# NingZhang1/pyscf_isdf

Hardware: AMD Instinct MI355X
Metric: isdf_build_plus_get_jk_wall_time (lower is better)
Workload: dtype f64

## Files before the change

### include/mi355_isdf.h

```cpp
#ifndef MI355_ISDF_H
#define MI355_ISDF_H

#include <stdint.h>

#ifdef __cplusplus
extern "C" {
#endif

typedef struct isdf_ctx* isdf_handle;

#define ISDF_OK 0
#define ISDF_ERR_ARG 1
#define ISDF_ERR_HIP 2
#define ISDF_ERR_LIB 3
#define ISDF_ERR_NUM 4

int isdf_abi_version(void);

int isdf_create(int device_id, isdf_handle* out);
int isdf_destroy(isdf_handle h);
int isdf_set_stream(isdf_handle h, void* hip_stream);
const char* isdf_last_error(isdf_handle h);
int64_t isdf_workspace_bytes(isdf_handle h);
int isdf_release_workspace(isdf_handle h);
// ... 58 lines not shown
int isdf_select_ip_gram(isdf_handle h, double* d_A, int m, int64_t ldA, int nip, double tol, double tie_rtol,
                        int panel, int64_t* d_piv, int32_t* rank);

int isdf_select_ip_cplx(isdf_handle h, const double* d_ao, int nao, int nh, int64_t ld,
                        int nblk, const int64_t* blk_off, const int32_t* nip,
                        double tol, double tie_rtol,
                        double* d_L, int64_t ldL, int64_t* d_piv, int32_t* rank);

int isdf_fit_from_chol(isdf_handle h, double* d_L, int k, int64_t m, int64_t ldL,
                       const int64_t* d_piv);

int isdf_fit_prepare(isdf_handle h, const double* d_ao, int nao, int64_t ld,
                     const int64_t* d_ip, int P, double reg_rel, double* d_aoP, double* d_chol,
                     double* reg_used);
int isdf_fit_apply(isdf_handle h, const double* d_chol, const double* d_aoP, int P, int nao,
                   const double* d_ao, int64_t ng, int64_t ld, int forward_only,
                   double* d_theta, int64_t ldt);
int isdf_fit_prepare_cplx(isdf_handle h, const double* d_ao, int nao, int nh, int64_t ld,
                          const int64_t* d_ip, int P, double reg_rel, double* d_aoP, double* d_chol,
                          double* reg_used);
int isdf_fit_apply_cplx(isdf_handle h, const double* d_chol, const double* d_aoP, int P, int nao, int nh,
                        const double* d_ao, int64_t ng, int64_t ld, int forward_only,
                        double* d_theta, int64_t ldt);
int isdf_fit_global(isdf_handle h, const double* d_ao, int nao, int64_t ngrids, int64_t ld,
                    const int64_t* d_ip, int P, double reg_rel, double* d_theta, int64_t ldt,
                    double* d_aoP, double* reg_used);

int isdf_gather_aoP(isdf_handle h, const double* d_ao, int nao, int64_t ld, const int64_t* d_ip, int P,
                    double* d_aoP);
int isdf_gram_sq(isdf_handle h, const double* d_aoP, int P, int nao, int nh, double* d_A);
int isdf_pair_gram_rows(isdf_handle h, const double* d_aoP, int P, int nao, int nh, const double* d_ao,
                        int64_t ng, int64_t ld, double* d_B, int64_t ldb);
int isdf_block_chol(isdf_handle h, const double* d_A, int P, int nblk, const int32_t* blk_off,
                    double shift_rel, double* d_D, double* shift_used);
int isdf_block_solve(isdf_handle h, const double* d_D, int P, int nblk, const int32_t* blk_off, int side,
                     int trans, double* d_X, int64_t n, int64_t ldx);
int isdf_block_invert(isdf_handle h, const double* d_D, int P, int nblk, const int32_t* blk_off, double* d_Dinv);
int isdf_block_apply(isdf_handle h, const double* d_Dinv, int64_t ldd, int nblk, const int32_t* blk_off,
                     double* d_X, int64_t n, int64_t ldx);
int isdf_pair_rows_block_apply(isdf_handle h, const double* d_aoP, int P, int nao, const double* d_ao, int64_t ng,
                               int64_t ld, const double* d_Dinv, int64_t ldd, int nblk, const int32_t* blk_off,
                               double* d_B, int64_t ldb);
int isdf_pair_rows_squared(isdf_handle h, const double* d_aoP, int rows, int nao, const double* d_ao, int64_t ng,
                           int64_t ld, int* squared);
int isdf_pair_rows_frontier(isdf_handle h, const double* d_aoP, int nnew, int nao, const double* d_ao, int64_t ng,
                            int64_t ld, int squared, const double* d_Dinv, int64_t ldd, int nblk, const int32_t* blk_off,
                            double* d_B, int64_t ldb, int have);

int isdf_gram_prod(isdf_handle h, const double* d_aoP, int P, int nao, const double* d_psiP, int nocc, double* d_A);
int isdf_pair_prod_rows(isdf_handle h, const double* d_aoP, int P, int nao, const double* d_psiP, int nocc,
                        const double* d_ao, int64_t ld, const double* d_psi, int64_t ldpsi, int64_t ng,
                        double* d_B, int64_t ldb);
int isdf_factor_solve_half(isdf_handle h, const double* d_fac, int P, int backward, double* d_X, int64_t n, int64_t ldx);
int isdf_gram_prod_cplx(isdf_handle h, const double* d_aoP, int P, int nao, int nh, const double* d_psiP, int npsi, int npsi_h,
                        double* d_A);
int isdf_pair_prod_rows_cplx(isdf_handle h, const double* d_aoP, int P, int nao, int nh, const double* d_psiP, int npsi,
                             int npsi_h, const double* d_ao, int64_t ld, const double* d_psi, int64_t ldpsi, int64_t ng,
                             double* d_B, int64_t ldb);

int isdf_shift_diag(isdf_handle h, double* d_A, int P, double shift_rel);
int isdf_chol_inplace(isdf_handle h, double* d_A, int P, double shift_rel, double* d_scratch, double* reg_used);

int isdf_factor_solve(isdf_handle h, const double* d_fac, int P, double* d_X, int64_t n, int64_t ldx);

int isdf_bj_probe_vectors(isdf_handle h, double* d_T, int n, const double* d_fac, const double* d_D, int P,
                          int nblk, const int32_t* blk_off);
int isdf_rows_combine(isdf_handle h, const double* d_E, int n, int64_t ldE, int rows, const double* d_Y,
                      int64_t ng, int64_t ldy, double* d_F, int64_t ldf, int accumulate);

int isdf_bj_probe_rows(isdf_handle h, double* d_T, int n, const double* d_fac, const double* d_D, int P, int nblk,
                       const int32_t* blk_off, const double* d_Yp, int64_t ng, int64_t ldy, double* d_F, int64_t ldf);

int isdf_gather_T(isdf_handle h, const double* d_L, int k, int64_t ldL, const int64_t* d_piv,
                  double* d_T);
int isdf_W_from_factor(isdf_handle h, const double* d_F, int P, int kind, double* d_M, int64_t ldm);

int isdf_coulomb_W(isdf_handle h, const double* d_theta, int P, int64_t ldt,
                   const int32_t mesh[3], const double a[9],
                   int row0, int nrows, int batch, int upper_only, double* d_W, int64_t ldw);
int isdf_coulG_half(isdf_handle h, const int32_t mesh[3], const double a[9], double* d_out);
int isdf_spectral_supported(isdf_handle h, const int32_t mesh[3], int batch, int* ok);
int isdf_spectral_rows(isdf_handle h, const double* d_in, int nrows, int64_t ld, const int32_t mesh[3], const int32_t* d_idx,
                       const double* d_scale, int npts, int batch, double* d_out, int64_t ldx);
int isdf_coulomb_rows(isdf_handle h, const double* d_in, int nrows, int64_t ld,
                      const int32_t mesh[3], const double a[9], int batch, double* d_out, int64_t ldo);
int isdf_symmetrize_upper(isdf_handle h, double* d_W, int P, int64_t ldw);
int isdf_symmetrize_mean(isdf_handle h, double* d_W, int P, int64_t ldw, int antisymmetric);

int isdf_get_j(isdf_handle h, const double* d_ao, int nao, int64_t ngrids, int64_t ld,
               const int32_t mesh[3], const double a[9],
               const double* d_dm, int nset, double* d_vj);
int isdf_rho(isdf_handle h, const double* d_ao, int nao, int64_t ng, int64_t ld,
             const double* d_dm, int nset, double* d_rho, int64_t ldrho);
int isdf_coulomb_potential(isdf_handle h, double* d_rho_inout, int nset, int64_t ldrho,
                           const int32_t mesh[3], const double a[9]);
int isdf_vj_from_vR(isdf_handle h, const double* d_ao, int nao, int64_t ng, int64_t ld,
                    const double* d_vR, int nset, int64_t ldv, double* d_vj);

int isdf_get_k_exact(isdf_handle h, const double* d_ao, int nao, int64_t ngrids, int64_t ld,
                     const double* d_C, int nocc, const int32_t mesh[3], const double a[9],
                     int i0, int ni, int max_rows, double* d_vk);

int isdf_get_k(isdf_handle h, const double* d_aoP, int P, int nao,
               const double* d_W, int64_t ldw, int row0, int nrows,
               const double* d_dm, int nset, double* d_vk);

int isdf_coulG_q(isdf_handle h, const int32_t mesh[3], const double a[9], const double q[3], int wrap_around,
                 double omega, double* d_out);

int isdf_coulomb_Wq(isdf_handle h, const double* d_theta, int P, int64_t ldt, const int32_t mesh[3],
                    const double* d_coulG, double weight, int row0, int nrows, int batch,
                    int upper_only, double* d_Wre, double* d_Wim, int64_t ldw);
int isdf_symmetrize_hermitian(isdf_handle h, double* d_Wre, double* d_Wim, int P, int64_t ldw);
int isdf_finish_Wq(isdf_handle h, const double* d_Wre, const double* d_Wim, int P, int64_t ldw,
                   const double* d_phase, double* d_Wc);
int isdf_get_k_pair(isdf_handle h, const double* d_A1, const double* d_A2, const double* d_D2,
                    const double* d_Wq, int P, int nao, double scale, double* d_vk);

int isdf_get_k_exact_kpt(isdf_handle h, const double* d_u1r, const double* d_u1i, int nao, int64_t ld1,
                         const double* d_m2r, const double* d_m2i, int nocc, int64_t ld2, const int32_t mesh[3],
                         const double* d_coulG, double weight, int i0, int ni, int max_rows, double* d_vk_re,
                         double* d_vk_im);

int isdf_coulomb_rows_q(isdf_handle h, const double* d_rows, int nrows, int64_t ld, const int32_t mesh[3],
                        const double* d_coulG, double* d_re, double* d_im);
int isdf_nyquist_spectra(isdf_handle h, const double* d_rows, int nrows, int64_t ld, const int32_t mesh[3], int axis,
                         double* d_re, double* d_im);
int isdf_zhadamard_planes(isdf_handle h, double* d_Ar, double* d_Ai, int64_t lda, const double* d_Br, const double* d_Bi,
                          int64_t ldb, int rows, int64_t cols);
int isdf_rho_k(isdf_handle h, const double* d_ur, const double* d_ui, int nao, int64_t ng, int64_t ld,
               const double* d_DTr, const double* d_DTi, double scale, double* d_rho);
int isdf_vj_k(isdf_handle h, const double* d_ur, const double* d_ui, int nao, int64_t ng, int64_t ld,
              const double* d_vR, double* d_vj_re, double* d_vj_im);

int isdf_pp_local_potential(isdf_handle h, int natm, const double* coords, const double* pp_par,
                            const int32_t mesh[3], const double a[9], double* d_vlocR);
int isdf_pp_projector_overlaps(isdf_handle h, const int32_t* atm, int natm, const int32_t* bas, int nbas,
                               const double* env, int nenv, const double* coords, const double kpt[3],
                               const int32_t* proj_tab, const double* proj_rl, int nproj,
                               const int32_t mesh[3], const double a[9], double* d_out);

int isdf_pp_local_force(isdf_handle h, const double* d_rho, int nset, int64_t ldrho, int natm, const double* coords,
                        const double* pp_par, const int32_t mesh[3], const double a[9], double* d_out);
int isdf_pp_projector_overlaps_ip(isdf_handle h, const int32_t* atm, int natm, const int32_t* bas, int nbas,
                                  const double* env, int nenv, const double* coords, const double kpt[3],
                                  const int32_t* proj_tab, const double* proj_rl, int nproj,
                                  const int32_t mesh[3], const double a[9], double* d_out);
int isdf_rowdot3(isdf_handle h, int M, int64_t K, double alpha, const double* d_A, int64_t lda, int64_t astride, const double* d_s,
                 const double* d_B, int64_t ldb, int accumulate, double* d_out, int64_t ldo);
int isdf_gga_aow(isdf_handle h, int M, int64_t K, const double* d_ao, int64_t ld, int64_t plane, const double* d_w, int64_t ldw,
                 double* d_Z, int64_t ldz, double* d_G, int64_t ldg, int64_t gstride);

int isdf_gemm_nn(isdf_handle h, int M, int64_t N, int K, double alpha, const double* d_A, int64_t lda, const double* d_B,
                 int64_t ldb, double beta, double* d_C, int64_t ldc);
int isdf_hadamard_rows(isdf_handle h, double* d_X, int64_t ldx, const double* d_Y, int64_t ldy, int rows, int64_t cols);

int isdf_uniform_grid(isdf_handle h, const int32_t mesh[3], const double a[9], double* d_coords_soa);
int isdf_rho_pair(isdf_handle h, const double* d_aoA, int nA, const double* d_aoB, int nB, int64_t ng, int64_t ld,
                  const double* d_dm, int nset, double* d_rho, int64_t ldrho);
int isdf_mg_embed_density(isdf_handle h, const double* d_field, int nset, const int32_t mesh_sub[3], double scale,
                          double* d_spec, const int32_t mesh[3], int accumulate);
int isdf_mg_restrict_potential(isdf_handle h, const double* d_spec, int nset, const int32_t mesh[3],
                               const int32_t mesh_sub[3], double scale, double* d_field);
int isdf_mg_coulomb_kernel(isdf_handle h, double* d_spec, int nset, const int32_t mesh[3], const double a[9]);
int isdf_lda_exchange(isdf_handle h, const double* d_rho, int64_t n, double* d_exc, double* d_vxc);
int isdf_lda_vwn_add(isdf_handle h, const double* d_rho, int64_t n, double* d_exc, double* d_vxc);
// ... 36 lines not shown
```

### pyscf_isdf_amd/backend.py

```python
import ctypes
import os
import numpy as np
import torch
from . import lib as _lib

_vp = ctypes.c_void_p


def _np_ptr(a):
    return a.ctypes.data_as(_vp)


class HipBackend:
    name = 'hip-gfx950'

    def __init__(self, device=0):
        if not torch.cuda.is_available():
            raise _lib.IsdfError('no GPU visible to torch; the ISDF path has no CPU fallback')
        self.device = torch.device('cuda', device)
        torch.cuda.set_device(self.device)
        self.handle = _lib.Handle(device)
        if os.environ.get('ISDF_TRSM') == 'subst':
            self.set_option('trsm_substitution', 1)
        if os.environ.get('ISDF_OWN_FFT') in ('0', '1', '2'):
# ... 309 lines not shown

    def shift_diag(self, A, shift_rel):
        self._stream()
        self.handle.call('isdf_shift_diag', self._p(A), A.shape[0], float(shift_rel))

    def chol_inplace(self, A, shift_rel, scratch=None):
        self._stream()
        reg = ctypes.c_double(0.0)
        assert scratch is None or scratch.numel() >= A.numel()
        self.handle.call('isdf_chol_inplace', self._p(A), A.shape[0], float(shift_rel),
                         self._p(scratch) if scratch is not None else None, ctypes.byref(reg))
        return reg.value

    def factor_solve(self, fac, X):
        self._stream()
        self.handle.call('isdf_factor_solve', self._p(fac), fac.shape[0], self._p(X), X.shape[1], X.stride(0))

    def bj_probe_rows(self, T, fac, D, blk_off, Yp, ng, F):
        self._stream()
        blk_off = np.ascontiguousarray(blk_off, dtype=np.int32)
        self.handle.call('isdf_bj_probe_rows', self._p(T), T.shape[0], self._p(fac), self._p(D), D.shape[0],
                         len(blk_off) - 1, _np_ptr(blk_off), self._p(Yp), int(ng), Yp.stride(0), self._p(F), F.stride(0))

    def bj_probe_vectors(self, T, fac, D, blk_off):
        self._stream()
        blk_off = np.ascontiguousarray(blk_off, dtype=np.int32)
        assert T.is_contiguous()
        self.handle.call('isdf_bj_probe_vectors', self._p(T), T.shape[0], self._p(fac), self._p(D), D.shape[0],
                         len(blk_off) - 1, _np_ptr(blk_off))

    def rows_combine(self, E, Y, F, accumulate=False):
        self._stream()
        assert E.stride(1) == 1 and Y.stride(1) == 1 and F.stride(1) == 1 and E.shape[1] == Y.shape[0]
        self.handle.call('isdf_rows_combine', self._p(E), E.shape[0], E.stride(0), E.shape[1], self._p(Y), Y.shape[1],
                         Y.stride(0), self._p(F), F.stride(0), int(bool(accumulate)))

    def gather_T(self, L, k, piv, T):
        self._stream()
        assert T.is_contiguous() and T.shape == (k, k)
        self.handle.call('isdf_gather_T', self._p(L), int(k), L.stride(0), self._p(piv), self._p(T))

    def W_from_factor(self, F, kind, M):
        self._stream()
        assert F.is_contiguous()
        self.handle.call('isdf_W_from_factor', self._p(F), M.shape[0], int(kind), self._p(M), M.stride(0))

    def fit_global(self, ao, ngrids, ip, reg_rel, theta, aoP):
        self._stream()
        assert ip.dtype == torch.int64 and aoP.is_contiguous()
        reg = ctypes.c_double(0.0)
        self.handle.call('isdf_fit_global', self._p(ao), ao.shape[0], int(ngrids), ao.stride(0), self._p(ip),
                         ip.numel(), float(reg_rel), self._p(theta), theta.stride(0), self._p(aoP), ctypes.byref(reg))
        return reg.value

    def coulomb_W(self, theta, mesh, a, row0, nrows, batch, W, upper_only=False):
        self._stream()
        mesh = np.ascontiguousarray(mesh, dtype=np.int32)
        a = np.ascontiguousarray(a, dtype=np.float64)
        self.handle.call('isdf_coulomb_W', self._p(theta), theta.shape[0], theta.stride(0), _np_ptr(mesh), _np_ptr(a),
                         int(row0), int(nrows), int(batch), int(bool(upper_only)), self._p(W), W.stride(0))

    def coulomb_rows(self, rows, mesh, a, batch, out=None):
        self._stream()
        out = rows if out is None else out
        mesh = np.ascontiguousarray(mesh, dtype=np.int32)
        a = np.ascontiguousarray(a, dtype=np.float64)
        self.handle.call('isdf_coulomb_rows', self._p(rows), rows.shape[0], rows.stride(0), _np_ptr(mesh), _np_ptr(a),
                         int(batch), self._p(out), out.stride(0))

    def spectral_supported(self, mesh, batch=512):
        ok = ctypes.c_int(0)
        mesh = np.ascontiguousarray(mesh, dtype=np.int32)
        self.handle.call('isdf_spectral_supported', _np_ptr(mesh), int(batch), ctypes.byref(ok))
        return bool(ok.value)

    def coulG_half(self, mesh, a):
        self._stream()
        mesh = np.ascontiguousarray(mesh, dtype=np.int32)
        a = np.ascontiguousarray(a, dtype=np.float64)
        out = self.empty((int(mesh[0]) * int(mesh[1]) * (int(mesh[2]) // 2 + 1),))
        self.handle.call('isdf_coulG_half', _np_ptr(mesh), _np_ptr(a), self._p(out))
        return self.to_host(out).reshape(int(mesh[0]), int(mesh[1]), int(mesh[2]) // 2 + 1)

    def spectral_rows(self, rows, mesh, idx, scale, out, batch=512):
        self._stream()
        mesh = np.ascontiguousarray(mesh, dtype=np.int32)
        assert rows.is_contiguous() and out.stride(1) == 1 and idx.dtype == torch.int32 and out.stride(0) % 2 == 0
        self.handle.call('isdf_spectral_rows', self._p(rows), rows.shape[0], rows.stride(0), _np_ptr(mesh), self._p(idx),
                         self._p(scale), int(idx.numel()), int(batch), self._p(out), out.stride(0))

    def symmetrize_upper(self, W):
        self._stream()
        self.handle.call('isdf_symmetrize_upper', self._p(W), W.shape[0], W.stride(0))

    def symmetrize_mean(self, W, antisymmetric=False):
        self._stream()
        self.handle.call('isdf_symmetrize_mean', self._p(W), W.shape[0], W.stride(0), int(bool(antisymmetric)))

    def get_j(self, ao, ngrids, mesh, a, dm, vj):
        self._stream()
        mesh = np.ascontiguousarray(mesh, dtype=np.int32)
        a = np.ascontiguousarray(a, dtype=np.float64)
        assert dm.is_contiguous() and vj.is_contiguous()
        self.handle.call('isdf_get_j', self._p(ao), ao.shape[0], int(ngrids), ao.stride(0), _np_ptr(mesh), _np_ptr(a),
                         self._p(dm), dm.shape[0], self._p(vj))

    def rho(self, ao, ng, dm, rho):
        self._stream()
        self.handle.call('isdf_rho', self._p(ao), ao.shape[0], int(ng), ao.stride(0), self._p(dm), dm.shape[0],
                         self._p(rho), rho.stride(0))

    def coulomb_potential(self, rho, mesh, a):
        self._stream()
        mesh = np.ascontiguousarray(mesh, dtype=np.int32)
        a = np.ascontiguousarray(a, dtype=np.float64)
        self.handle.call('isdf_coulomb_potential', self._p(rho), rho.shape[0], rho.stride(0), _np_ptr(mesh), _np_ptr(a))

    def vj_from_vR(self, ao, ng, vR, vj):
        self._stream()
        self.handle.call('isdf_vj_from_vR', self._p(ao), ao.shape[0], int(ng), ao.stride(0), self._p(vR), vR.shape[0],
                         vR.stride(0), self._p(vj))

    def get_k(self, aoP, W, row0, nrows, dm, vk):
        self._stream()
        assert aoP.is_contiguous() and dm.is_contiguous() and vk.is_contiguous()
        self.handle.call('isdf_get_k', self._p(aoP), aoP.shape[0], aoP.shape[1], self._p(W), W.stride(0), int(row0),
                         int(nrows), self._p(dm), dm.shape[0], self._p(vk))

    def get_k_exact(self, ao, ngrids, C, mesh, a, i0, ni, max_rows, vk):
        self._stream()
        mesh = np.ascontiguousarray(mesh, dtype=np.int32)
        a = np.ascontiguousarray(a, dtype=np.float64)
        assert C.is_contiguous() and vk.is_contiguous()
        self.handle.call('isdf_get_k_exact', self._p(ao), ao.shape[0], int(ngrids), ao.stride(0), self._p(C), C.shape[1],
                         _np_ptr(mesh), _np_ptr(a), int(i0), int(ni), int(max_rows), self._p(vk))

    def gemm_nn(self, A, B, C, alpha=1.0, beta=0.0):
        self._stream()
        self.handle.call('isdf_gemm_nn', A.shape[0], B.shape[1], A.shape[1], float(alpha), self._p(A), A.stride(0), self._p(B),
                         B.stride(0), float(beta), self._p(C), C.stride(0))

    def hadamard_rows(self, X, Y):
        self._stream()
        self.handle.call('isdf_hadamard_rows', self._p(X), X.stride(0), self._p(Y), Y.stride(0), X.shape[0], X.shape[1])

    def gemm_nt(self, A, B, C, alpha=1.0, beta=0.0, kscale=None):
        self._stream()
        M, K = A.shape
        N = B.shape[0]
        assert B.shape[1] == K and tuple(C.shape) == (M, N) and A.stride(1) == 1 and B.stride(1) == 1 and C.stride(1) == 1
        ks = self._p(kscale) if kscale is not None else _vp(0)
        self.handle.call('isdf_gemm_nt', M, N, K, float(alpha), self._p(A), A.stride(0), self._p(B), B.stride(0), ks,
                         float(beta), self._p(C), C.stride(0))

    def gemm_nt_had3(self, A, H, B3, C3, alpha=1.0, beta=0.0):
        self._stream()
        M, K = A.shape
        N = B3.shape[1]
        assert tuple(B3.shape) == (3, N, K) and tuple(C3.shape) == (3, M, N) and A.stride(1) == 1 and B3.stride(2) == 1 and C3.stride(2) == 1
        assert H is None or (tuple(H.shape) == (M, K) and H.stride(1) == 1)
        self.handle.call('isdf_gemm_nt_had3', M, N, K, float(alpha), self._p(A), A.stride(0), self._p(H) if H is not None else _vp(0),
                         H.stride(0) if H is not None else 0, self._p(B3), B3.stride(1), B3.stride(0), float(beta), self._p(C3),
                         C3.stride(1), C3.stride(0))

    def gemm_nn_had(self, A, H, B, C, alpha=1.0, beta=0.0):
        self._stream()
        M, K = A.shape
        N = B.shape[1]
        assert tuple(B.shape) == (K, N) and tuple(H.shape) == (K, N) and tuple(C.shape) == (M, N)
        assert A.stride(1) == 1 and H.stride(1) == 1 and B.stride(1) == 1 and C.stride(1) == 1
        self.handle.call('isdf_gemm_nn_had', M, N, K, float(alpha), self._p(A), A.stride(0), self._p(H), H.stride(0), self._p(B),
                         B.stride(0), float(beta), self._p(C), C.stride(0))
# ... 283 lines not shown
```

### pyscf_isdf_amd/csrc/common.h

```cpp
#pragma once
#include <hip/hip_runtime.h>
#include <rocblas/rocblas.h>
#include <rocsolver/rocsolver.h>
#include <hipfft/hipfft.h>
#include <cstdint>
#include <cstdio>
#include <cstring>
#include <string>
#include <vector>
#include <map>
#include "../../include/mi355_isdf.h"

struct FftPlan {
  hipfftHandle fwd = 0, bwd = 0;
  size_t work_bytes = 0;
};

struct ProfRec {
  hipEvent_t e0 = nullptr, e1 = nullptr;
};
struct ProfEntry {
  std::vector<ProfRec> recs;
  double work = 0.0;
  double ms = 0.0;
  int64_t launches = 0;
};

struct WsKernel {
  double alpha = 0.0;
  double ak[9] = {0};
  int mesh[3] = {0, 0, 0};
  double maxq[3] = {0, 0, 0};
  const double* vq = nullptr;
};

struct isdf_ctx {
  int profiling = 0;
  std::map<std::string, ProfEntry> prof;
  int device = 0;
  hipStream_t stream = nullptr;
  rocblas_handle blas = nullptr;
  std::string err;
  std::map<std::vector<int>, FftPlan> plans;
  std::map<std::string, std::pair<void*, size_t>> ws;
  int num_cu = 256;
  int trsm_substitution = 0;
  int own_fft = 2;
  int gemm_nn_own = 0;
  int attr_gemm_b = 0, attr_gemm_nn = 0, attr_gemm_nn_had = 0, attr_gram_tri = 0, attr_herm = 0;
  int cand_gram = 1;
  int conv_pipe = 1;
  int conv_sub_rows = 0;
  int gram_pivot_tpb = 256;
  int gram_compact = 1;
  int gram_compact_permille = 875;
  int block_apply_waves = 16;
  int block_apply_reg = 1;
  double coul_omega = 0.0;
  double coul_rc = 0.0;
  int coul_sphere = 0;
  WsKernel wsk;
};

int isdf_fail(isdf_handle h, int code, const char* fmt, ...);
void* isdf_ws(isdf_handle h, const char* name, size_t bytes);
int isdf_get_plan(isdf_handle h, const int32_t mesh[3], int batch, FftPlan** out);
int get_coulG_half(isdf_handle h, const int32_t mesh[3], const double a[9], double extra_scale, double** out);
bool conv_rows_own_supported(const int32_t mesh[3], int nb);
bool conv_rows_q_own_supported(isdf_handle h, const int32_t mesh[3], int nb);
bool spectral_rows_own_supported(isdf_handle h, const int32_t mesh[3], int nb);
int spectral_rows_own(isdf_handle h, const double* d_in, int nb, const int32_t mesh[3], const int32_t* d_idx, const double* d_scale,
                      int npts, double* d_out, int64_t ldx, HIP_vector_type<double, 2u>* zbuf);
int conv_rows_q_own(isdf_handle h, const double* d_in, double* d_re, double* d_im, int nb, const int32_t mesh[3], const double* tab,
                    double2* zhalf, double2* zfull);
int conv_rows_own(isdf_handle h, const double* d_in, double* d_out, int nb, const int32_t mesh[3], const double* cg,
                  double2* zbuf);

#define HIP_TRY(h, expr)                                                                    \
  do {                                                                                      \
    hipError_t e_ = (expr);                                                                 \
    if (e_ != hipSuccess)                                                                   \
      return isdf_fail(h, ISDF_ERR_HIP, "%s:%d %s -> %s", __FILE__, __LINE__, #expr,        \
                       hipGetErrorString(e_));                                              \
  } while (0)
#define BLAS_TRY(h, expr)                                                                   \
  do {                                                                                      \
    rocblas_status s_ = (expr);                                                             \
    if (s_ != rocblas_status_success)                                                       \
      return isdf_fail(h, ISDF_ERR_LIB, "%s:%d %s -> rocblas status %d", __FILE__, __LINE__, \
                       #expr, (int)s_);                                                     \
  } while (0)
#define FFT_TRY(h, expr)                                                                    \
  do {                                                                                      \
    hipfftResult r_ = (expr);                                                               \
    if (r_ != HIPFFT_SUCCESS)                                                               \
      return isdf_fail(h, ISDF_ERR_LIB, "%s:%d %s -> hipfft result %d", __FILE__, __LINE__,  \
                       #expr, (int)r_);                                                     \
  } while (0)
#define KERNEL_CHECK(h) HIP_TRY(h, hipGetLastError())
#define ARG_CHECK(h, cond)                                                                  \
  do {                                                                                      \
    if (!(cond)) return isdf_fail(h, ISDF_ERR_ARG, "%s:%d argument check failed: %s",       \
                                  __FILE__, __LINE__, #cond);                               \
  } while (0)

static inline int64_t cdiv(int64_t a, int64_t b) { return (a + b - 1) / b; }

struct ProfScope {
  isdf_handle h;
  ProfRec rec;
  ProfEntry* ent = nullptr;
  ProfScope(isdf_handle h_, const char* name, double work, int64_t launches = 1) : h(h_) {
    if (!h || !h->profiling) return;
    ent = &h->prof[name];
    ent->work += work;
    ent->launches += launches;
    if (hipEventCreate(&rec.e0) != hipSuccess || hipEventCreate(&rec.e1) != hipSuccess) { ent = nullptr; return; }
    (void)hipEventRecord(rec.e0, h->stream);
  }
  ~ProfScope() {
    if (!ent) return;
    (void)hipEventRecord(rec.e1, h->stream);
    ent->recs.push_back(rec);
  }
};

int gemm_nt_f64(isdf_handle h, int M, int N, int64_t K, double alpha, const double* A, int64_t lda,
                const double* B, int64_t ldb, double beta, double* C, int64_t ldc);
int gemm_nt_f64_scaled(isdf_handle h, int M, int N, int64_t K, double alpha, const double* A, int64_t lda,
                       const double* B, int64_t ldb, const double* kscale, double beta, double* C,
                       int64_t ldc);
int trsm_lower_left(isdf_handle h, bool trans, int m, int64_t n, const double* L, int64_t ldl, double* X, int64_t ldx);
int trsm_lower_right(isdf_handle h, bool trans, int m, int64_t n, const double* L, int64_t ldl, double* X, int64_t ldx);
int block_forward_solve(isdf_handle h, const double* D, int64_t ldd, int nblk, const int32_t* blk_off_host, double* X,
                        int64_t ldx, int64_t n);
int block_apply_inverse(isdf_handle h, const double* Dinv, int64_t ldd, int nblk, const int32_t* blk_off_host, double* X,
                        int64_t ldx, int64_t n, bool square_input = false);
int transpose_rm(isdf_handle h, const double* src, int64_t lds, int64_t rows, int64_t cols, double* dst, int64_t ldd);
int tri_left(isdf_handle h, bool trans, int m, int64_t n, const double* L, int64_t ldl, double* X, int64_t ldx);
int tri_right(isdf_handle h, bool trans, int m, int64_t n, const double* L, int64_t ldl, double* X, int64_t ldx);
bool gemm_nn_f64_supported(isdf_handle h, int64_t M, int64_t N, int64_t K, const double* A, int64_t lda, const double* B,
                           int64_t ldb);
int gemm_nn_f64(isdf_handle h, int64_t M, int64_t N, int64_t K, const double* A, int64_t lda, const double* B, int64_t ldb,
                double* C, int64_t ldc, bool square);
int gemm_rm(isdf_handle h, char opA, char opB, int64_t M, int64_t N, int64_t K, double alpha,
            const double* A, int64_t lda, const double* B, int64_t ldb, double beta, double* C,
            int64_t ldc);

__host__ __device__ inline int64_t gram_tri_row(int64_t r) {
  const int64_t tm = r >> 8;
  return 32768 * tm * (tm + 1) + (r & 255) * ((tm + 1) << 8);
}
static inline int64_t gram_tri_size(int64_t m) { return m > 0 ? gram_tri_row(m - 1) + (((m - 1) >> 8) + 1) * 256 : 0; }
struct GramTriUnit { int blk, tm, tn, pad; };
int gram_tri_blocks(isdf_handle h, const double* X, int64_t ldx, int K, const GramTriUnit* d_units, int64_t nunits,
                    const int64_t* d_blk_off, int64_t row0, const int64_t* d_tri_off, double* S, double flop);
```

### pyscf_isdf_amd/csrc/coulomb.hip

```cpp
#include "common.h"

namespace {

struct Recip { double b[9]; };
__device__ inline double g2_of(int ix, int iy, int iz, int n0, int n1, int n2, const Recip& r) {
  const double fx = (ix < (n0 + 1) / 2) ? ix : ix - n0;
  const double fy = (iy < (n1 + 1) / 2) ? iy : iy - n1;
  const double fz = (iz < (n2 + 1) / 2) ? iz : iz - n2;
  const double gx = fx * r.b[0] + fy * r.b[3] + fz * r.b[6];
  const double gy = fx * r.b[1] + fy * r.b[4] + fz * r.b[7];
  const double gz = fx * r.b[2] + fy * r.b[5] + fz * r.b[8];
  return gx * gx + gy * gy + gz * gz;
}

__device__ inline double range_factor(double g2, double omega) {
  if (omega == 0.0) return 1.0;
  const double e = exp(-0.25 * g2 / (omega * omega));
  return omega > 0.0 ? e : 1.0 - e;
}
__device__ inline double kernel_value(double g2, double omega, double rc) {
  const double fourpi = 4.0 * 3.14159265358979323846;
  if (rc > 0.0) return g2 == 0.0 ? 0.5 * fourpi * rc * rc : fourpi / g2 * (1.0 - cos(sqrt(g2) * rc));
  return g2 == 0.0 ? 0.0 : fourpi / g2 * range_factor(g2, omega);
}
// ... 270 lines not shown
    if (rc) return rc;
  }
  return ISDF_OK;
}

extern "C" int isdf_coulomb_potential(isdf_handle h, double* d_rho, int nset, int64_t ldrho,
                                      const int32_t mesh[3], const double a[9]) {
  if (!h) return ISDF_ERR_ARG;
  ARG_CHECK(h, d_rho && mesh && a && nset > 0);
  const int64_t G = (int64_t)mesh[0] * mesh[1] * mesh[2];
  const int64_t gc = (int64_t)mesh[0] * mesh[1] * (mesh[2] / 2 + 1);
  ARG_CHECK(h, ldrho == G);
  const double det = a[0] * (a[4] * a[8] - a[5] * a[7]) - a[1] * (a[3] * a[8] - a[5] * a[6]) +
                     a[2] * (a[3] * a[7] - a[4] * a[6]);
  double* cg = nullptr;
  int rc = get_coulG_half(h, mesh, a, fabs(det) / (double)G, &cg);
  if (rc) return rc;
  double2* Z = (double2*)isdf_ws(h, "coul_Z", sizeof(double2) * (size_t)nset * gc);
  if (!Z) return ISDF_ERR_HIP;
  return convolve_rows(h, d_rho, d_rho, nset, mesh, cg, Z);
}

extern "C" int isdf_coulomb_rows(isdf_handle h, const double* d_in, int nrows, int64_t ld,
                                 const int32_t mesh[3], const double a[9], int batch, double* d_out,
                                 int64_t ldo) {
  if (!h) return ISDF_ERR_ARG;
  ARG_CHECK(h, d_in && d_out && mesh && a && nrows >= 0 && batch > 0);
  const int64_t G = (int64_t)mesh[0] * mesh[1] * mesh[2];
  const int64_t gc = (int64_t)mesh[0] * mesh[1] * (mesh[2] / 2 + 1);
  ARG_CHECK(h, ld == G && ldo == G);
  if (nrows == 0) return ISDF_OK;
  if (batch > nrows) batch = nrows;
  double* cg = nullptr;
  int rc = get_coulG_half(h, mesh, a, 1.0, &cg);
  if (rc) return rc;
  double2* Z = (double2*)isdf_ws(h, "coul_Z", sizeof(double2) * (size_t)batch * gc);
  if (!Z) return ISDF_ERR_HIP;
  for (int r = 0; r < nrows; r += batch) {
    const int nb = std::min(batch, nrows - r);
    rc = convolve_rows(h, d_in + (int64_t)r * ld, d_out + (int64_t)r * ldo, nb, mesh, cg, Z);
    if (rc) return rc;
  }
  return ISDF_OK;
}

extern "C" int isdf_coulG_half(isdf_handle h, const int32_t mesh[3], const double a[9], double* d_out) {
  if (!h) return ISDF_ERR_ARG;
  ARG_CHECK(h, mesh && a && d_out);
  double* cg = nullptr;
  int rc = get_coulG_half(h, mesh, a, 1.0, &cg);
  if (rc) return rc;
  const int64_t gc = (int64_t)mesh[0] * mesh[1] * (mesh[2] / 2 + 1);
  HIP_TRY(h, hipMemcpyAsync(d_out, cg, sizeof(double) * gc, hipMemcpyDeviceToDevice, h->stream));
  return ISDF_OK;
}

extern "C" int isdf_spectral_supported(isdf_handle h, const int32_t mesh[3], int batch, int* ok) {
  if (!h) return ISDF_ERR_ARG;
  ARG_CHECK(h, mesh && ok && batch > 0);
  *ok = spectral_rows_own_supported(h, mesh, batch) ? 1 : 0;
  return ISDF_OK;
}

extern "C" int isdf_spectral_rows(isdf_handle h, const double* d_in, int nrows, int64_t ld, const int32_t mesh[3],
                                  const int32_t* d_idx, const double* d_scale, int npts, int batch, double* d_out, int64_t ldx) {
  if (!h) return ISDF_ERR_ARG;
  ARG_CHECK(h, d_in && d_out && mesh && d_idx && d_scale && nrows >= 0 && batch > 0 && npts > 0);
  const int64_t G = (int64_t)mesh[0] * mesh[1] * mesh[2];
  const int64_t gc = (int64_t)mesh[0] * mesh[1] * (mesh[2] / 2 + 1);
  ARG_CHECK(h, ld == G && npts <= gc);
  if (nrows == 0) return ISDF_OK;
  if (batch > nrows) batch = nrows;
  if (!spectral_rows_own_supported(h, mesh, batch))
    return isdf_fail(h, ISDF_ERR_ARG, "isdf_spectral_rows: mesh %d x %d x %d is not covered by the plane FFT", mesh[0], mesh[1], mesh[2]);
  double2* Z = (double2*)isdf_ws(h, "coul_Z", sizeof(double2) * (size_t)batch * gc);
  if (!Z) return ISDF_ERR_HIP;
  for (int r = 0; r < nrows; r += batch) {
    const int nb = std::min(batch, nrows - r);
    int rc = spectral_rows_own(h, d_in + (int64_t)r * ld, nb, mesh, d_idx, d_scale, npts, d_out + (int64_t)r * ldx, ldx, Z);
    if (rc) return rc;
  }
  return ISDF_OK;
}
```

### pyscf_isdf_amd/csrc/fft_conv.hip

```cpp
#include "common.h"
#include <type_traits>

namespace {

constexpr int TPB = 256;
constexpr int MAXSTAGE = 12;

struct Axis {
  int n;
  int nstage;
  int radix[MAXSTAGE];
  const double2* tw;
};

__device__ inline double2 cadd(double2 a, double2 b) { return make_double2(a.x + b.x, a.y + b.y); }
__device__ inline double2 csub(double2 a, double2 b) { return make_double2(a.x - b.x, a.y - b.y); }
__device__ inline double2 cmul(double2 a, double2 b) { return make_double2(a.x * b.x - a.y * b.y, a.x * b.y + a.y * b.x); }
template <int SIGN>
__device__ inline double2 mul_si(double2 a) { return SIGN > 0 ? make_double2(-a.y, a.x) : make_double2(a.y, -a.x); }
template <int SIGN>
__device__ inline double2 twid(const double2* __restrict__ tw, int idx) {
  double2 w = tw[idx];
  if (SIGN > 0) w.y = -w.y;
  return w;
// ... 432 lines not shown
    if ((l & 1) == 0) r = make_double2(0.5 * (zk.x + zn.x), 0.5 * (zk.y - zn.y));
    else r = make_double2(0.5 * (zk.y + zn.y), -0.5 * (zk.x - zn.x));
    dstc[c] = r;
  }
}

template <int ZCT>
__global__ __launch_bounds__(TPB) void z_c2r_fast_kernel(const double2* __restrict__ in, double* __restrict__ out,
                                                         int64_t nlines, Axis ax) {
  extern __shared__ double2 lds[];
  const int n = ax.n, nh = n / 2 + 1;
  constexpr int Ls = ZCT + 1;
  double2* x = lds;
  double2* tw = lds + n * Ls;
  for (int k = threadIdx.x; k < n; k += TPB) tw[k] = ax.tw[k];
  const int64_t line0 = (int64_t)blockIdx.x * 2 * ZCT;
  const int nl = (int)min((int64_t)2 * ZCT, nlines - line0);
  const int M = (nl + 1) / 2;
  const double2* src = in + line0 * nh;
  const float inv_nh = 1.0f / (float)nh;
  for (int c = threadIdx.x; c < M * nh; c += TPB) {
    const int m = (int)(((float)c + 0.5f) * inv_nh), k = c - m * nh;
    double2 a = src[(int64_t)(2 * m) * nh + k];
    double2 b = (2 * m + 1 < nl) ? src[(int64_t)(2 * m + 1) * nh + k] : make_double2(0.0, 0.0);
    const bool selfconj = (k == 0) || (2 * k == n);
    if (selfconj) { a.y = 0.0; b.y = 0.0; }
    x[k * Ls + m] = make_double2(a.x - b.y, a.y + b.x);
    if (!selfconj) x[(n - k) * Ls + m] = make_double2(a.x + b.y, -a.y + b.x);
  }
  __syncthreads();
  fft_fast<1, ZCT>(x, ax, Ls, tw);
  double* dst = out + line0 * n;
  const float inv_n = 1.0f / (float)n;
  for (int c = threadIdx.x; c < nl * n; c += TPB) {
    const int l = (int)(((float)c + 0.5f) * inv_n), e = c - l * n;
    dst[c] = ((const double*)(x + e * Ls + (l >> 1)))[l & 1];
  }
}

template <int MODE, int ZCT>
__global__ __launch_bounds__(TPB) void strided_fft_fast_kernel(double2* __restrict__ data, int64_t os, int64_t es, int Mtot,
                                                               Axis ax, int ntile, const double* __restrict__ table) {
  extern __shared__ double2 lds[];
  const int n = ax.n;
  double2* x = lds;
  double2* tw = lds + n * ZCT;
  for (int k = threadIdx.x; k < n; k += TPB) tw[k] = ax.tw[k];
  const int nouter = gridDim.x / ntile;
  const int64_t outer = (MODE == 2) ? blockIdx.x % nouter : blockIdx.x / ntile;
  const int m0 = (int)((MODE == 2) ? blockIdx.x / nouter : blockIdx.x % ntile) * ZCT;
  const int M = min(ZCT, Mtot - m0);
  double2* base = data + outer * os + m0;
  for (int c = threadIdx.x; c < n * ZCT; c += TPB) {
    const int e = c / ZCT, m = c & (ZCT - 1);
    if (m < M) x[c] = base[(int64_t)e * es + m];
  }
  __syncthreads();
  if (MODE == 1) {
    fft_fast<1, ZCT>(x, ax, ZCT, tw);
  } else {
    fft_fast<-1, ZCT>(x, ax, ZCT, tw);
    if (MODE == 2) {
      const double* tb = table + m0;
      for (int c = threadIdx.x; c < n * ZCT; c += TPB) {
        const int e = c / ZCT, m = c & (ZCT - 1);
        if (m < M) {
          const double g = tb[(int64_t)e * es + m];
          double2 v = x[c];
          v.x *= g;
          v.y *= g;
          x[c] = v;
        }
      }
      __syncthreads();
      fft_fast<1, ZCT>(x, ax, ZCT, tw);
    }
  }
  for (int c = threadIdx.x; c < n * ZCT; c += TPB) {
    const int e = c / ZCT, m = c & (ZCT - 1);
    if (m < M) base[(int64_t)e * es + m] = x[c];
  }
}

constexpr int TPBP = 1024;
constexpr int PLANE_ENTRIES = 10240;
constexpr int PIPE_NT = 768;

template <int SIGN, int NT, int N, int RA, int RB, int MMAX>
__device__ __forceinline__ void fft_plane_fixed(double2* buf, int Ls, int M, const double2* tw) {
  static_assert(RA * RB == N, "two stages");
  stage<SIGN, RA, NT, ((N / RA) * MMAX + NT - 1) / NT, true, AnyLines>(buf, N, N, 1, Ls, M, tw, opaque_tid());
  stage<SIGN, RB, NT, ((N / RB) * MMAX + NT - 1) / NT, true, AnyLines>(buf, N, N / RA, RA, Ls, M, tw, opaque_tid());
}

struct PlaneAny {
  static constexpr int NT = TPBP, PER = PLANE_ENTRIES / TPBP;
  static constexpr int KS_HALF = PER, KS_PAIR = PER / 2 + 1, KS_FULL = PER;
  int n1, n2, n2h, npair;
  __device__ PlaneAny(const Axis& az, const Axis& ay) : n1(ay.n), n2(az.n), n2h(az.n / 2 + 1), npair((ay.n + 1) / 2) {}
  __device__ static int tid() { return threadIdx.x; }
  template <int SIGN, bool FULL>
  __device__ __forceinline__ static void transform(double2* buf, const Axis& ax, int Ls, int M, const double2* tw) {
    fft<SIGN, NT, PER, false, AnyLines>(buf, ax, Ls, M, tw);
  }
};
template <int N, int RA, int RB>
struct PlaneSquare {
  static constexpr int NT = PIPE_NT, n1 = N, n2 = N, n2h = N / 2 + 1, npair = (N + 1) / 2;
  static constexpr int KS_HALF = (n1 * n2h + NT - 1) / NT, KS_PAIR = (npair * n2h + NT - 1) / NT, KS_FULL = (N * N + NT - 1) / NT;
  constexpr PlaneSquare() = default;
  __device__ static int tid() { return opaque_tid(); }
  template <int SIGN, bool FULL>
  __device__ __forceinline__ static void transform(double2* buf, const Axis&, int Ls, int M, const double2* tw) {
    fft_plane_fixed<SIGN, NT, N, RA, RB, FULL ? N : N / 2 + 1>(buf, Ls, M, tw);
  }
};

__device__ inline double zero_of(const double*) { return 0.0; }
__device__ inline double2 zero_of(const double2*) { return make_double2(0.0, 0.0); }
template <int NT, int NPRE, class T>
__device__ __forceinline__ void prefetch(T (&pre)[NPRE], const T* __restrict__ src, int count, int tid) {
#pragma unroll
  for (int u = 0; u < NPRE; ++u) {
    const int c = tid + u * NT;
    pre[u] = c < count ? src[c] : zero_of(src);
  }
}

template <class D>
__device__ __forceinline__ void plane_fwd_body(const D d, double2* lds, int Lz, int bufsz, const Axis& az, const Axis& ay,
                                               double2* __restrict__ dst, double2 (&r)[D::KS_HALF]) {
  double2* x = lds;
  const double2* twz = lds + bufsz;
  const double2* twy = twz + d.n2;
  d.template transform<-1, false>(x, az, Lz, d.npair, twz);
  int tid = D::tid();
  const float inv_nh = 1.0f / (float)d.n2h;
#pragma unroll
  for (int u = 0; u < D::KS_HALF; ++u) {
    const int c = tid + u * D::NT;
    if (c < d.n1 * d.n2h) {
      const int l = fdiv(c, inv_nh), k = c - l * d.n2h;
      const int m = l >> 1;
      r[u] = separate_pair(x[k * Lz + m], x[(k == 0 ? 0 : d.n2 - k) * Lz + m], l & 1);
    }
  }
  __syncthreads();
#pragma unroll
  for (int u = 0; u < D::KS_HALF; ++u) {
    const int c = tid + u * D::NT;
    if (c < d.n1 * d.n2h) x[c] = r[u];
  }
  __syncthreads();
  d.template transform<-1, false>(x, ay, d.n2h, d.n2h, twy);
  tid = D::tid();
  for (int c = tid; c < d.n1 * d.n2h; c += D::NT) dst[c] = x[c];
}

template <class D>
__device__ __forceinline__ void plane_inv_body(const D d, double2* lds, int Lz, int bufsz, const Axis& az, const Axis& ay,
                                               double* __restrict__ dst, double2 (&za)[D::KS_PAIR], double2 (&zb)[D::KS_PAIR]) {
  double2* x = lds;
  const double2* twz = lds + bufsz;
  const double2* twy = twz + d.n2;
  d.template transform<1, false>(x, ay, d.n2h, d.n2h, twy);
  int tid = D::tid();
// ... 451 lines not shown

int conv_rows_own(isdf_handle h, const double* d_in, double* d_out, int nb, const int32_t mesh[3], const double* cg,
                  double2* zbuf) {
  const int n0 = mesh[0], n1 = mesh[1], n2 = mesh[2], n2h = n2 / 2 + 1;
  Axis ax[3];
  if (int rc = make_axes(h, mesh, ax, "conv_rows_own")) return rc;
  const int64_t gc = (int64_t)n0 * n1 * n2h;
  const int64_t nlines = (int64_t)nb * n0 * n1;
  ARG_CHECK(h, nlines * 4 < 2147483647LL && (int64_t)nb * cdiv((int64_t)n1 * n2h, 1) < 2147483647LL);
  const int LP = lines_per_tile(n2, 1);
  const int ZY = lines_per_tile(n1, 0), ZX = lines_per_tile(n0, 0);
  if (LP < 1 || ZY < 1 || ZX < 1) return isdf_fail(h, ISDF_ERR_ARG, "conv_rows_own: mesh too large for the LDS tiles");
  const int64_t G = (int64_t)n0 * n1 * n2;
  const int FZ = fast_lines(n2), FY = fast_lines(n1), FX = fast_lines(n0);
  const bool smooth = smooth235(ax[0]) && smooth235(ax[1]) && smooth235(ax[2]);
  const PlaneGeo geo = (h->own_fft == 2 && smooth && FX >= 1) ? plane_geometry(n1, n2, false) : PlaneGeo{0, 0, 0};
  ProfScope ps(h, geo.bytes ? "coulomb_conv_own_3pass[byte]" : "coulomb_conv_own_5pass[byte]", 32.0 * (double)G * nb,
               geo.bytes ? 3 : 5);
  if (geo.bytes) {
    const int sub = h->conv_sub_rows > 0 ? std::min(nb, h->conv_sub_rows) : nb;
    for (int r0 = 0; r0 < nb; r0 += sub) {
      const int nr = std::min(sub, nb - r0);
      double2* zb = zbuf + (int64_t)r0 * gc;
      const int nplanes = (int)((int64_t)nr * n0);
      if (int rc = launch_plane_fwd(h, d_in + (int64_t)r0 * G, zb, ax, geo, nplanes, PIPE_ANY)) return rc;
      launch_strided<2>(h, true, FX, zb, nr, gc, (int64_t)n1 * n2h, n1 * n2h, ax[0], cg);
      if (int rc = launch_plane_inv(h, zb, d_out + (int64_t)r0 * G, ax, geo, nplanes, PIPE_ANY)) return rc;
    }
    KERNEL_CHECK(h);
    return ISDF_OK;
  }
  const bool fast = smooth && FZ >= 1 && FY >= 1 && FX >= 1;
  const int Lz = fast ? FZ : LP, Ly = fast ? FY : ZY, Lx = fast ? FX : ZX;
  launch_z<true>(h, fast, Lz, d_in, zbuf, nlines, ax[2]);
  launch_strided<0>(h, fast, Ly, zbuf, (int64_t)nb * n0, (int64_t)n1 * n2h, (int64_t)n2h, n2h, ax[1], nullptr);
  launch_strided<2>(h, fast, Lx, zbuf, nb, gc, (int64_t)n1 * n2h, n1 * n2h, ax[0], cg);
  launch_strided<1>(h, fast, Ly, zbuf, (int64_t)nb * n0, (int64_t)n1 * n2h, (int64_t)n2h, n2h, ax[1], nullptr);
  launch_z<false>(h, fast, Lz, zbuf, d_out, nlines, ax[2]);
  KERNEL_CHECK(h);
  return ISDF_OK;
}

__global__ void spectral_pack_kernel(const double2* __restrict__ z, int64_t gc, const int32_t* __restrict__ idx,
                                     const double* __restrict__ scale, int npts, double2* __restrict__ out, int64_t ldx2) {
  const int64_t j = (int64_t)blockIdx.x * blockDim.x + threadIdx.x;
  if (j >= ldx2) return;
  const int row = blockIdx.y;
  double2 v = make_double2(0.0, 0.0);
  if (j < npts) {
    const double2 t = z[(int64_t)row * gc + idx[j]];
    const double s = scale[j];
    v = make_double2(t.x * s, t.y * s);
  }
  out[(int64_t)row * ldx2 + j] = v;
}

bool spectral_rows_own_supported(isdf_handle h, const int32_t mesh[3], int nb) {
  if (h->own_fft != 2 || !conv_rows_own_supported(mesh, nb)) return false;
  Axis ax[3];
  for (int d = 0; d < 3; ++d)
    if (!factorise(mesh[d], &ax[d]) || !smooth235(ax[d])) return false;
  return fast_lines(mesh[0]) >= 1 && plane_geometry(mesh[1], mesh[2], false).bytes != 0;
}

int spectral_rows_own(isdf_handle h, const double* d_in, int nb, const int32_t mesh[3], const int32_t* d_idx,
                      const double* d_scale, int npts, double* d_out, int64_t ldx, double2* zbuf) {
  const int n0 = mesh[0], n1 = mesh[1], n2 = mesh[2], n2h = n2 / 2 + 1;
  Axis ax[3];
  if (int rc = make_axes(h, mesh, ax, "spectral_rows_own")) return rc;
  const int64_t gc = (int64_t)n0 * n1 * n2h;
  const PlaneGeo geo = plane_geometry(n1, n2, false);
  const int FX = fast_lines(n0);
  ARG_CHECK(h, geo.bytes && FX >= 1 && (int64_t)nb * n0 < 2147483647LL && nb <= 65535 && (ldx & 1) == 0 && ldx >= 2 * (int64_t)npts);
  ProfScope ps(h, "spectral_rows_own[byte]", (8.0 * (double)n0 * n1 * n2 + 8.0 * (double)ldx) * nb, 3);
  if (int rc = launch_plane_fwd(h, d_in, zbuf, ax, geo, (int)((int64_t)nb * n0), PIPE_ANY)) return rc;
  launch_strided<0>(h, true, FX, zbuf, nb, gc, (int64_t)n1 * n2h, n1 * n2h, ax[0], nullptr);
  const int64_t ldx2 = ldx / 2;
  spectral_pack_kernel<<<dim3((unsigned)cdiv(ldx2, 256), (unsigned)nb), dim3(256), 0, h->stream>>>(zbuf, gc, d_idx, d_scale, npts,
                                                                                                  (double2*)d_out, ldx2);
  KERNEL_CHECK(h);
  return ISDF_OK;
}

bool conv_rows_q_own_supported(isdf_handle h, const int32_t mesh[3], int nb) {
  if (!h->own_fft) return false;
  if (nb < 1 || nb > 65535 || (int64_t)nb * mesh[0] >= 2147483647LL) return false;
  Axis ax[3];
  for (int d = 0; d < 3; ++d)
    if (mesh[d] < 2 || mesh[d] > 1024 || !factorise(mesh[d], &ax[d]) || !smooth235(ax[d])) return false;
  return fast_lines(mesh[0]) >= 1 && plane_geometry(mesh[1], mesh[2], false).bytes && plane_geometry(mesh[1], mesh[2], true).bytes;
}

int conv_rows_q_own(isdf_handle h, const double* d_in, double* d_re, double* d_im, int nb, const int32_t mesh[3],
                    const double* tab, double2* zhalf, double2* zfull) {
  const int n0 = mesh[0], n1 = mesh[1], n2 = mesh[2], n2h = n2 / 2 + 1;
  Axis ax[3];
  if (int rc = make_axes(h, mesh, ax, "conv_rows_q_own")) return rc;
  const int64_t G = (int64_t)n0 * n1 * n2, gc = (int64_t)n0 * n1 * n2h;
  const PlaneGeo geo_r = plane_geometry(n1, n2, false), geo_c = plane_geometry(n1, n2, true);
  const int FX = fast_lines(n0);
  ARG_CHECK(h, geo_r.bytes && geo_c.bytes && FX >= 1 && (int64_t)nb * n0 < 2147483647LL && nb <= 65535);
  ProfScope ps(h, "coulomb_conv_q_own[byte]", 64.0 * (double)G * nb, 5);
  const int nplanes = (int)((int64_t)nb * n0);
  if (int rc = launch_plane_fwd(h, d_in, zhalf, ax, geo_r, nplanes, PIPE_Q_MAX)) return rc;
  launch_strided<0>(h, true, FX, zhalf, nb, gc, (int64_t)n1 * n2h, n1 * n2h, ax[0], nullptr);
  expand_mul_kernel<<<dim3((unsigned)cdiv(G, 256), (unsigned)nb), dim3(256), 0, h->stream>>>(zhalf, zfull, tab, n0, n1, n2,
                                                                                            1.0 / (double)G);
  launch_strided<1>(h, true, FX, zfull, nb, G, (int64_t)n1 * n2, n1 * n2, ax[0], nullptr);
  if (int rc = launch_plane_c2c_inv(h, zfull, d_re, d_im, ax, geo_c, nplanes)) return rc;
  KERNEL_CHECK(h);
  return ISDF_OK;
}
```

### pyscf_isdf_amd/csrc/fit.hip

```cpp
#include "common.h"
#include <cstdlib>

namespace {

__global__ void gather_T_kernel(const double* __restrict__ L, int64_t ldL,
                                const int64_t* __restrict__ piv, int k, double* __restrict__ T) {
  const int s = blockIdx.x * blockDim.x + threadIdx.x;
  const int t = blockIdx.y;
  if (s >= k) return;
  T[(int64_t)t * k + s] = (s >= t) ? L[(int64_t)t * ldL + piv[s]] : 0.0;
}

__global__ void square_kernel(double* __restrict__ x, int64_t rows, int64_t cols, int64_t ld) {
  const int64_t c = (int64_t)blockIdx.x * blockDim.x + threadIdx.x;
  const int64_t r = blockIdx.y;
  if (c >= cols) return;
  const double v = x[r * ld + c];
  x[r * ld + c] = v * v;
}

__global__ void square_add_kernel(double* __restrict__ x, int64_t ld, const double* __restrict__ y, int64_t ldy,
                                  int64_t cols) {
  const int64_t c = (int64_t)blockIdx.x * blockDim.x + threadIdx.x;
  const int64_t r = blockIdx.y;
// ... 279 lines not shown
    }
    __syncthreads();
    if (live) {
      const double* y = Y + (int64_t)p0 * ldy + g;
#pragma unroll 8
      for (int pp = 0; pp < np; ++pp) {
        const double v = y[(int64_t)pp * ldy];
#pragma unroll
        for (int j = 0; j < 8; ++j) acc[j] = fma(sE[j][pp], v, acc[j]);
      }
    }
  }
  if (live)
    for (int j = 0; j < n; ++j) F[(int64_t)j * ldf + g] = accumulate ? F[(int64_t)j * ldf + g] + acc[j] : acc[j];
}

__global__ void add_diag_const_kernel(double* __restrict__ A, int n, int64_t ld, double v) {
  const int i = blockIdx.x * blockDim.x + threadIdx.x;
  if (i < n) A[(int64_t)i * ld + i] += v;
}
}

extern "C" int isdf_block_chol(isdf_handle h, const double* d_A, int P, int nblk, const int32_t* blk_off,
                               double shift_rel, double* d_D, double* shift_used) {
  if (!h) return ISDF_ERR_ARG;
  ARG_CHECK(h, d_A && d_D && blk_off && P > 0 && nblk > 0 && blk_off[0] == 0 && blk_off[nblk] == P && shift_rel >= 0);
  int* info = (int*)isdf_ws(h, "fit_info", 256);
  if (!info) return ISDF_ERR_HIP;
  double* maxdiag = (double*)(info + 16);
  HIP_TRY(h, hipMemsetAsync(d_D, 0, sizeof(double) * (size_t)P * P, h->stream));
  hipLaunchKernelGGL(max_diag_kernel, dim3(1), dim3(256), 0, h->stream, d_A, P, maxdiag);
  double md = 0.0;
  HIP_TRY(h, hipMemcpyAsync(&md, maxdiag, sizeof(double), hipMemcpyDeviceToHost, h->stream));
  HIP_TRY(h, hipStreamSynchronize(h->stream));
  double worst = 0.0;
  for (int b = 0; b < nblk; ++b) {
    const int off = blk_off[b], nb = blk_off[b + 1] - off;
    if (nb <= 0) continue;
    ARG_CHECK(h, nb <= 65535);
    double reg = shift_rel;
    int h_info = 1;
    for (int attempt = 0; attempt < 6 && h_info != 0; ++attempt) {
      hipLaunchKernelGGL(copy_block_kernel, dim3((unsigned)cdiv(nb, 128), (unsigned)nb), dim3(128), 0, h->stream, d_A, P,
                         off, nb, d_D);
      if (reg > 0)
        hipLaunchKernelGGL(add_diag_const_kernel, dim3((unsigned)cdiv(nb, 256)), dim3(256), 0, h->stream,
                           d_D + (int64_t)off * P + off, nb, (int64_t)P, reg * md);
      KERNEL_CHECK(h);
      BLAS_TRY(h, rocsolver_dpotrf(h->blas, rocblas_fill_upper, nb, d_D + (int64_t)off * P + off, P, info));
      HIP_TRY(h, hipMemcpyAsync(&h_info, info, sizeof(int), hipMemcpyDeviceToHost, h->stream));
      HIP_TRY(h, hipStreamSynchronize(h->stream));
      if (h_info == 0) { worst = std::max(worst, reg); break; }
      reg = (reg > 0.0) ? reg * 100.0 : 1e-14;
    }
    if (h_info != 0)
      return isdf_fail(h, ISDF_ERR_NUM, "diagonal block %d of A_PP is not positive definite even with shift %g * max diag "
                       "(minor %d of %d)", b, reg / 100.0, h_info, nb);
  }
  if (shift_used) *shift_used = worst;
  return ISDF_OK;
}

extern "C" int isdf_block_solve(isdf_handle h, const double* d_D, int P, int nblk, const int32_t* blk_off, int side,
                                int trans, double* d_X, int64_t n, int64_t ldx) {
  if (!h) return ISDF_ERR_ARG;
  ARG_CHECK(h, d_D && d_X && blk_off && P > 0 && nblk > 0 && n > 0 && (side == 0 || side == 1) && (trans == 0 || trans == 1));
  ARG_CHECK(h, n < 2147483647LL && ldx < 2147483647LL);
  if (side == 0 && trans == 0 && !h->trsm_substitution) {
    ARG_CHECK(h, blk_off[0] == 0 && blk_off[nblk] <= P);
    return block_forward_solve(h, d_D, P, nblk, blk_off, d_X, ldx, n);
  }
  for (int b = 0; b < nblk; ++b) {
    const int off = blk_off[b], nb = blk_off[b + 1] - off;
    if (nb <= 0) continue;
    const double* Db = d_D + (int64_t)off * P + off;
    const int rc = (side == 0) ? tri_left(h, trans != 0, nb, n, Db, P, d_X + (int64_t)off * ldx, ldx)
                               : tri_right(h, trans != 0, nb, n, Db, P, d_X + off, ldx);
    if (rc) return rc;
  }
  return ISDF_OK;
}

namespace {
__global__ void block_identity_kernel(double* __restrict__ E, int P, const int32_t* __restrict__ blk_of_row) {
  const int64_t i = (int64_t)blockIdx.x * blockDim.x + threadIdx.x;
  if (i < (int64_t)P * P) E[i] = (i / P == i % P) ? 1.0 : 0.0;
  (void)blk_of_row;
}
}

extern "C" int isdf_block_invert(isdf_handle h, const double* d_D, int P, int nblk, const int32_t* blk_off, double* d_Dinv) {
  if (!h) return ISDF_ERR_ARG;
  ARG_CHECK(h, d_D && d_Dinv && blk_off && P > 0 && nblk > 0 && blk_off[0] == 0 && blk_off[nblk] <= P);
  hipLaunchKernelGGL(block_identity_kernel, dim3((unsigned)cdiv((int64_t)P * P, 256)), dim3(256), 0, h->stream, d_Dinv, P,
                     (const int32_t*)nullptr);
  KERNEL_CHECK(h);
  return block_forward_solve(h, d_D, P, nblk, blk_off, d_Dinv, P, P);
}

extern "C" int isdf_block_apply(isdf_handle h, const double* d_Dinv, int64_t ldd, int nblk, const int32_t* blk_off,
                                double* d_X, int64_t n, int64_t ldx) {
  if (!h) return ISDF_ERR_ARG;
  ARG_CHECK(h, d_Dinv && d_X && blk_off && nblk > 0 && n > 0 && ldx >= n && blk_off[0] == 0 && blk_off[nblk] <= ldd);
  return block_apply_inverse(h, d_Dinv, ldd, nblk, blk_off, d_X, ldx, n);
}

extern "C" int isdf_pair_rows_block_apply(isdf_handle h, const double* d_aoP, int P, int nao, const double* d_ao, int64_t ng,
                                          int64_t ld, const double* d_Dinv, int64_t ldd, int nblk, const int32_t* blk_off,
                                          double* d_B, int64_t ldb) {
  if (!h) return ISDF_ERR_ARG;
  ARG_CHECK(h, d_aoP && d_ao && d_Dinv && d_B && blk_off && P > 0 && nao > 0 && ng > 0 && ld >= ng && ldb >= ng && nblk > 0);
  ARG_CHECK(h, blk_off[0] == 0 && blk_off[nblk] == P);
  const bool own = gemm_nn_f64_supported(h, P, ng, nao, d_aoP, nao, d_ao, ld);
  int rc = product_rows(h, P, ng, nao, d_aoP, d_ao, ld, d_B, ldb, own);
  if (rc) return rc;
  return block_apply_inverse(h, d_Dinv, ldd, nblk, blk_off, d_B, ldb, ng, !own);
}

extern "C" int isdf_pair_rows_squared(isdf_handle h, const double* d_aoP, int rows, int nao, const double* d_ao, int64_t ng,
                                      int64_t ld, int* squared) {
  if (!h) return ISDF_ERR_ARG;
  ARG_CHECK(h, d_aoP && d_ao && squared && rows > 0 && nao > 0 && ng > 0 && ld >= ng);
  *squared = gemm_nn_f64_supported(h, rows, ng, nao, d_aoP, nao, d_ao, ld) ? 1 : 0;
  return ISDF_OK;
}

extern "C" int isdf_pair_rows_frontier(isdf_handle h, const double* d_aoP, int nnew, int nao, const double* d_ao, int64_t ng,
                                       int64_t ld, int squared, const double* d_Dinv, int64_t ldd, int nblk,
                                       const int32_t* blk_off, double* d_B, int64_t ldb, int have) {
  if (!h) return ISDF_ERR_ARG;
  ARG_CHECK(h, d_ao && d_B && nnew >= 0 && nnew <= 65535 && have >= 0 && nblk >= 0 && nao > 0 && ng > 0 && ld >= ng && ldb >= ng);
  ARG_CHECK(h, (nnew == 0 || d_aoP) && (nblk == 0 || (d_Dinv && blk_off && blk_off[0] == 0 && blk_off[nblk] <= have + nnew)));
  if (nnew > 0) {
    double* rows = d_B + (int64_t)have * ldb;
    int rc = squared ? product_rows(h, nnew, ng, nao, d_aoP, d_ao, ld, rows, ldb, true)
                     : gemm_rm(h, 'N', 'N', nnew, ng, nao, 1.0, d_aoP, nao, d_ao, ld, 0.0, rows, ldb);
    if (rc) return rc;
  }
  if (nblk == 0) return ISDF_OK;
  return block_apply_inverse(h, d_Dinv, ldd, nblk, blk_off, d_B, ldb, ng, !squared);
}

extern "C" int isdf_shift_diag(isdf_handle h, double* d_A, int P, double shift_rel) {
  if (!h) return ISDF_ERR_ARG;
  ARG_CHECK(h, d_A && P > 0 && shift_rel >= 0);
  if (shift_rel == 0.0) return ISDF_OK;
  int* info = (int*)isdf_ws(h, "fit_info", 256);
  if (!info) return ISDF_ERR_HIP;
  double* maxdiag = (double*)(info + 16);
  hipLaunchKernelGGL(max_diag_kernel, dim3(1), dim3(256), 0, h->stream, d_A, P, maxdiag);
  hipLaunchKernelGGL(add_diag_kernel, dim3((unsigned)cdiv(P, 256)), dim3(256), 0, h->stream, d_A, P, maxdiag, shift_rel);
  KERNEL_CHECK(h);
  return ISDF_OK;
}

extern "C" int isdf_chol_inplace(isdf_handle h, double* d_A, int P, double shift_rel, double* d_scratch,
                                 double* reg_used) {
  if (!h) return ISDF_ERR_ARG;
  ARG_CHECK(h, d_A && P > 0 && shift_rel >= 0);
  int* info = (int*)isdf_ws(h, "fit_info", 256);
  double* keep = d_scratch ? d_scratch : (double*)isdf_ws(h, "chol_keep", sizeof(double) * (size_t)P * P);
  if (!info || !keep) return ISDF_ERR_HIP;
  double* maxdiag = (double*)(info + 16);
  HIP_TRY(h, hipMemcpyAsync(keep, d_A, sizeof(double) * (size_t)P * P, hipMemcpyDeviceToDevice, h->stream));
  double reg = shift_rel;
  for (int attempt = 0; attempt < 5; ++attempt) {
    if (attempt > 0)
      HIP_TRY(h, hipMemcpyAsync(d_A, keep, sizeof(double) * (size_t)P * P, hipMemcpyDeviceToDevice, h->stream));
    if (reg > 0) {
      hipLaunchKernelGGL(max_diag_kernel, dim3(1), dim3(256), 0, h->stream, d_A, P, maxdiag);
      hipLaunchKernelGGL(add_diag_kernel, dim3((unsigned)cdiv(P, 256)), dim3(256), 0, h->stream, d_A, P, maxdiag, reg);
      KERNEL_CHECK(h);
    }
    { ProfScope ps(h, "rocsolver_dpotrf[flop]", (double)P * P * P / 3.0);
      BLAS_TRY(h, rocsolver_dpotrf(h->blas, rocblas_fill_upper, P, d_A, P, info)); }
    int h_info = 0;
    HIP_TRY(h, hipMemcpyAsync(&h_info, info, sizeof(int), hipMemcpyDeviceToHost, h->stream));
    HIP_TRY(h, hipStreamSynchronize(h->stream));
    if (h_info == 0) {
      if (reg_used) *reg_used = reg;
// ... 226 lines not shown
```

### pyscf_isdf_amd/csrc/trsm.hip

```cpp
#include "common.h"
#include <cstdlib>

namespace {

constexpr int SB = 64;

template <bool TRANS>
__global__ __launch_bounds__(256) void subst_kernel(const double* __restrict__ L, int64_t ldl, int nb,
                                                    double* __restrict__ X, int64_t ldx, int64_t n) {
  const int64_t c = (int64_t)blockIdx.x * 256 + threadIdx.x;
  if (c >= n) return;
  double x[SB];
#pragma unroll
  for (int i = 0; i < SB; ++i) x[i] = (i < nb) ? X[(int64_t)i * ldx + c] : 0.0;
  if (!TRANS) {
#pragma unroll
    for (int i = 0; i < SB; ++i) {
      if (i < nb) {
        double s = x[i];
#pragma unroll
        for (int k = 0; k < i; ++k) s = fma(-L[(int64_t)i * ldl + k], x[k], s);
        x[i] = s / L[(int64_t)i * ldl + i];
      }
    }
  } else {
#pragma unroll
    for (int i = SB - 1; i >= 0; --i) {
      if (i < nb) {
        double s = x[i];
#pragma unroll
        for (int k = i + 1; k < SB; ++k)
          if (k < nb) s = fma(-L[(int64_t)k * ldl + i], x[k], s);
        x[i] = s / L[(int64_t)i * ldl + i];
      }
    }
  }
#pragma unroll
  for (int i = 0; i < SB; ++i)
    if (i < nb) X[(int64_t)i * ldx + c] = x[i];
}

__global__ void transpose_kernel(const double* __restrict__ src, int64_t lds, int64_t rows, int64_t cols,
                                 double* __restrict__ dst, int64_t ldd) {
  __shared__ double tile[32][33];
  const int64_t r0 = (int64_t)blockIdx.y * 32, c0 = (int64_t)blockIdx.x * 32;
  const int tx = threadIdx.x, ty = threadIdx.y;
  for (int i = ty; i < 32; i += 8) {
    const int64_t r = r0 + i, c = c0 + tx;
    tile[i][tx] = (r < rows && c < cols) ? src[r * lds + c] : 0.0;
  }
  __syncthreads();
  for (int i = ty; i < 32; i += 8) {
    const int64_t r = c0 + i, c = r0 + tx;
    if (r < cols && c < rows) dst[r * ldd + c] = tile[tx][i];
  }
}

__global__ __launch_bounds__(256) void block_forward_kernel(const double* __restrict__ D, int64_t ldd,
                                                            const int32_t* __restrict__ blk_off,
                                                            double* __restrict__ X, int64_t ldx, int64_t n) {
  const int b = blockIdx.y;
  const int off = blk_off[b], m = blk_off[b + 1] - off;
  if (m <= 0) return;
  const int64_t c = (int64_t)blockIdx.x * 256 + threadIdx.x;
  if (c >= n) return;
  const double* Db = D + (int64_t)off * ldd + off;
  double* Xb = X + (int64_t)off * ldx + c;
  const int nsub = (m + 63) >> 6;
  double x[SB];
  for (int j = 0; j < nsub; ++j) {
    const int nbj = min(SB, m - j * SB);
    const double* Lj = Db + (int64_t)(j * SB) * ldd;
#pragma unroll
    for (int q = 0; q < SB; ++q) x[q] = (q < nbj) ? Xb[(int64_t)(j * SB + q) * ldx] : 0.0;
    for (int r0 = 0; r0 < j * SB; r0 += 8) {
      double v[8];
#pragma unroll
      for (int t = 0; t < 8; ++t) v[t] = Xb[(int64_t)(r0 + t) * ldx];
#pragma unroll
      for (int q = 0; q < SB; ++q) {
        if (q < nbj) {
          const double* Lq = Lj + (int64_t)q * ldd + r0;
#pragma unroll
          for (int t = 0; t < 8; ++t) x[q] = fma(-Lq[t], v[t], x[q]);
        }
      }
    }
    const double* Ld = Lj + j * SB;
#pragma unroll
    for (int q = 0; q < SB; ++q) {
      if (q < nbj) {
        double s_ = x[q];
#pragma unroll
        for (int k = 0; k < q; ++k) s_ = fma(-Ld[(int64_t)q * ldd + k], x[k], s_);
        x[q] = s_ / Ld[(int64_t)q * ldd + q];
      }
    }
#pragma unroll
    for (int q = 0; q < SB; ++q)
      if (q < nbj) Xb[(int64_t)(j * SB + q) * ldx] = x[q];
  }
}

int subst(isdf_handle h, bool trans, const double* L, int64_t ldl, int nb, double* X, int64_t ldx, int64_t n) {
  ProfScope ps(h, trans ? "trsm_subst_kernel<true>[flop]" : "trsm_subst_kernel<false>[flop]", (double)nb * nb * (double)n);
  const dim3 grid((unsigned)cdiv(n, 256));
  if (trans) hipLaunchKernelGGL(subst_kernel<true>, grid, dim3(256), 0, h->stream, L, ldl, nb, X, ldx, n);
  else hipLaunchKernelGGL(subst_kernel<false>, grid, dim3(256), 0, h->stream, L, ldl, nb, X, ldx, n);
  KERNEL_CHECK(h);
  return ISDF_OK;
}

}

typedef double d4v __attribute__((ext_vector_type(4)));
template <int TN, bool SQ>
__global__ __launch_bounds__(256) void block_apply_mfma_kernel(const double* __restrict__ Dinv, int64_t ldd,
                                                               const int32_t* __restrict__ blk_off, double* __restrict__ X,
                                                               int64_t ldx, int64_t n) {
  extern __shared__ double sB[];
  constexpr int LDB = TN + 2;
  const int b = blockIdx.y;
  const int off = blk_off[b], m = blk_off[b + 1] - off;
  if (m <= 0) return;
  const int mpad = (m + 31) & ~31;
  const int64_t c0 = (int64_t)blockIdx.x * TN;
  const int ncol = (int)min((int64_t)TN, n - c0);
  double* Xb = X + (int64_t)off * ldx + c0;
  for (int idx = threadIdx.x; idx < mpad * TN; idx += 256) {
    const int r = idx / TN, c = idx - r * TN;
    double v = (r < m && c < ncol) ? Xb[(int64_t)r * ldx + c] : 0.0;
    if (SQ) v = v * v;
    sB[r * LDB + c] = v;
  }
  __syncthreads();
  const int wave = threadIdx.x >> 6, lane = threadIdx.x & 63;
  const int fr = lane & 15, fk = lane >> 4;
  for (int rt = wave; rt < (m + 15) / 16; rt += 4) {
    d4v acc[TN / 16];
#pragma unroll
    for (int ct = 0; ct < TN / 16; ++ct) acc[ct] = (d4v){0.0, 0.0, 0.0, 0.0};
    const int arow = rt * 16 + fr;
    const bool rowok = arow < m;
    const double* pa = Dinv + (int64_t)(off + (rowok ? arow : 0)) * ldd + off + 8 * fk;
    const double* pb = sB + (8 * fk) * LDB + fr;
    const int kend = min(mpad, ((rt + 1) * 16 + 31) & ~31);
    double a_cur[8], a_nxt[8];
#pragma unroll
// ... 117 lines not shown

template <int NT, int NCT>
static int block_apply_reg_launch(isdf_handle h, const double* Dinv, int64_t ldd, int nblk, const int32_t* d_off, double* X,
                                  int64_t ldx, int64_t n, bool sq) {
  constexpr int TN = 16 * NCT;
  constexpr int NTHREADS = 64 * ((NT + 1) / 2);
  static_assert(NTHREADS % TN == 0 && (16 * NT * TN) % NTHREADS == 0, "tile elements must divide evenly over the threads");
  const size_t lds = (size_t)16 * NT * (TN + 2) * sizeof(double);
  const int64_t ntile = (n + TN - 1) / TN;
  const unsigned gx = (unsigned)std::max<int64_t>(1, std::min<int64_t>(ntile, ((int64_t)h->num_cu * h->block_apply_waves + nblk - 1) / nblk));
  if (sq) {
    if (lds > 64 * 1024)
      HIP_TRY(h, hipFuncSetAttribute((const void*)&block_apply_reg_kernel<NT, NCT, true>, hipFuncAttributeMaxDynamicSharedMemorySize, 160 * 1024));
    hipLaunchKernelGGL(HIP_KERNEL_NAME(block_apply_reg_kernel<NT, NCT, true>), dim3(gx, (unsigned)nblk), dim3(NTHREADS), lds, h->stream,
                       Dinv, ldd, d_off, X, ldx, n);
  } else {
    if (lds > 64 * 1024)
      HIP_TRY(h, hipFuncSetAttribute((const void*)&block_apply_reg_kernel<NT, NCT, false>, hipFuncAttributeMaxDynamicSharedMemorySize, 160 * 1024));
    hipLaunchKernelGGL(HIP_KERNEL_NAME(block_apply_reg_kernel<NT, NCT, false>), dim3(gx, (unsigned)nblk), dim3(NTHREADS), lds, h->stream,
                       Dinv, ldd, d_off, X, ldx, n);
  }
  KERNEL_CHECK(h);
  return ISDF_OK;
}

template <int TN, bool SQ>
static hipError_t block_apply_lds_attr() {
  return hipFuncSetAttribute((const void*)&block_apply_mfma_kernel<TN, SQ>, hipFuncAttributeMaxDynamicSharedMemorySize, 160 * 1024);
}

int block_apply_inverse(isdf_handle h, const double* Dinv, int64_t ldd, int nblk, const int32_t* blk_off_host, double* X,
                        int64_t ldx, int64_t n, bool square_input) {
  ARG_CHECK(h, Dinv && X && blk_off_host && nblk > 0 && n > 0 && nblk <= 65535);
  int mmax = 0;
  for (int b = 0; b < nblk; ++b) mmax = std::max(mmax, blk_off_host[b + 1] - blk_off_host[b]);
  const int mpad = (mmax + 31) & ~31;
  ARG_CHECK(h, mmax > 0);
  const bool reg = h->block_apply_reg && mmax <= 256;
  const int nt = (mmax + 15) / 16;
  int tn = 0;
  const char* label;
  if (reg) {
    label = nt <= 8 ? "block_apply_reg_kernel<8,2>[byte]" : nt <= 10 ? "block_apply_reg_kernel<10,2>[byte]"
          : nt <= 12 ? "block_apply_reg_kernel<12,2>[byte]" : "block_apply_reg_kernel<16,1>[byte]";
  } else if ((size_t)mpad * (64 + 2) * sizeof(double) <= 52 * 1024) {
    tn = 64; label = "block_apply_mfma_kernel<64>[byte]";
  } else if ((size_t)mpad * (32 + 2) * sizeof(double) <= 80 * 1024) {
    tn = 32; label = "block_apply_mfma_kernel<32>[byte]";
  } else {
    ARG_CHECK(h, (size_t)mpad * (16 + 2) * sizeof(double) <= 160 * 1024);
    tn = 16; label = "block_apply_mfma_kernel<16>[byte]";
  }
  int32_t* d_off = (int32_t*)isdf_ws(h, "trsm_blk_off", sizeof(int32_t) * (size_t)(nblk + 1));
  if (!d_off) return ISDF_ERR_HIP;
  HIP_TRY(h, hipMemcpyAsync(d_off, blk_off_host, sizeof(int32_t) * (size_t)(nblk + 1), hipMemcpyHostToDevice, h->stream));
  ProfScope ps(h, label, 16.0 * (double)blk_off_host[nblk] * (double)n);
  if (reg) {
    if (nt <= 8) return block_apply_reg_launch<8, 2>(h, Dinv, ldd, nblk, d_off, X, ldx, n, square_input);
    if (nt <= 10) return block_apply_reg_launch<10, 2>(h, Dinv, ldd, nblk, d_off, X, ldx, n, square_input);
    if (nt <= 12) return block_apply_reg_launch<12, 2>(h, Dinv, ldd, nblk, d_off, X, ldx, n, square_input);
    return block_apply_reg_launch<16, 1>(h, Dinv, ldd, nblk, d_off, X, ldx, n, square_input);
  }
#define ISDF_BA_LAUNCH(TN_, SQ_)                                                                                       \
  do {                                                                                                                 \
    if ((size_t)mpad * (TN_ + 2) * sizeof(double) > 64 * 1024) {                                                       \
      HIP_TRY(h, (block_apply_lds_attr<TN_, SQ_>()));                                                                  \
    }                                                                                                                  \
    hipLaunchKernelGGL(HIP_KERNEL_NAME(block_apply_mfma_kernel<TN_, SQ_>), dim3((unsigned)cdiv(n, TN_), (unsigned)nblk),   \
                       dim3(256), (size_t)mpad * (TN_ + 2) * sizeof(double), h->stream, Dinv, ldd, d_off, X, ldx, n);  \
  } while (0)
  if (tn == 64) {
    if (square_input) ISDF_BA_LAUNCH(64, true); else ISDF_BA_LAUNCH(64, false);
  } else if (tn == 32) {
    if (square_input) ISDF_BA_LAUNCH(32, true); else ISDF_BA_LAUNCH(32, false);
  } else {
    if (square_input) ISDF_BA_LAUNCH(16, true); else ISDF_BA_LAUNCH(16, false);
  }
#undef ISDF_BA_LAUNCH
  KERNEL_CHECK(h);
  return ISDF_OK;
}

int block_forward_solve(isdf_handle h, const double* D, int64_t ldd, int nblk, const int32_t* blk_off_host, double* X,
                        int64_t ldx, int64_t n) {
  ARG_CHECK(h, D && X && blk_off_host && nblk > 0 && n > 0 && nblk <= 65535);
  int32_t* d_off = (int32_t*)isdf_ws(h, "trsm_blk_off", sizeof(int32_t) * (size_t)(nblk + 1));
  if (!d_off) return ISDF_ERR_HIP;
  HIP_TRY(h, hipMemcpyAsync(d_off, blk_off_host, sizeof(int32_t) * (size_t)(nblk + 1), hipMemcpyHostToDevice, h->stream));
  double rows2 = 0.0;
  for (int b = 0; b < nblk; ++b) rows2 += (double)(blk_off_host[b + 1] - blk_off_host[b]) * (blk_off_host[b + 1] - blk_off_host[b]);
  ProfScope ps(h, "block_forward_kernel[byte]", 16.0 * (double)blk_off_host[nblk] * (double)n);
  (void)rows2;
  hipLaunchKernelGGL(block_forward_kernel, dim3((unsigned)cdiv(n, 256), (unsigned)nblk), dim3(256), 0, h->stream, D, ldd, d_off,
                     X, ldx, n);
  KERNEL_CHECK(h);
  return ISDF_OK;
}

int transpose_rm(isdf_handle h, const double* src, int64_t lds, int64_t rows, int64_t cols, double* dst, int64_t ldd) {
  ARG_CHECK(h, src && dst && rows > 0 && cols > 0 && lds >= cols && ldd >= rows);
  hipLaunchKernelGGL(transpose_kernel, dim3((unsigned)cdiv(cols, 32), (unsigned)cdiv(rows, 32)), dim3(32, 8), 0, h->stream,
                     src, lds, rows, cols, dst, ldd);
  KERNEL_CHECK(h);
  return ISDF_OK;
}

int trsm_lower_left(isdf_handle h, bool trans, int m, int64_t n, const double* L, int64_t ldl, double* X, int64_t ldx) {
  ARG_CHECK(h, L && X && m > 0 && n > 0 && ldl >= m && ldx >= n);
  const int PB = 512;
  int rc;
  if (!trans) {
    for (int r0 = 0; r0 < m; r0 += PB) {
      const int r1 = std::min(m, r0 + PB);
      if (r0 > 0) {
        rc = gemm_rm(h, 'N', 'N', r1 - r0, n, r0, -1.0, L + (int64_t)r0 * ldl, ldl, X, ldx, 1.0, X + (int64_t)r0 * ldx, ldx);
        if (rc) return rc;
      }
      for (int s0 = r0; s0 < r1; s0 += SB) {
        const int s1 = std::min(r1, s0 + SB);
        if (s0 > r0) {
          rc = gemm_rm(h, 'N', 'N', s1 - s0, n, s0 - r0, -1.0, L + (int64_t)s0 * ldl + r0, ldl, X + (int64_t)r0 * ldx, ldx,
                       1.0, X + (int64_t)s0 * ldx, ldx);
          if (rc) return rc;
        }
        rc = subst(h, false, L + (int64_t)s0 * ldl + s0, ldl, s1 - s0, X + (int64_t)s0 * ldx, ldx, n);
        if (rc) return rc;
      }
    }
  } else {
    const int npan = (int)cdiv(m, PB);
    for (int p = npan - 1; p >= 0; --p) {
      const int r0 = p * PB, r1 = std::min(m, r0 + PB);
      if (r1 < m) {
        rc = gemm_rm(h, 'T', 'N', r1 - r0, n, m - r1, -1.0, L + (int64_t)r1 * ldl + r0, ldl, X + (int64_t)r1 * ldx, ldx, 1.0,
                     X + (int64_t)r0 * ldx, ldx);
        if (rc) return rc;
      }
      const int nsb = (int)cdiv(r1 - r0, SB);
      for (int q = nsb - 1; q >= 0; --q) {
        const int s0 = r0 + q * SB, s1 = std::min(r1, s0 + SB);
        if (s1 < r1) {
          rc = gemm_rm(h, 'T', 'N', s1 - s0, n, r1 - s1, -1.0, L + (int64_t)s1 * ldl + s0, ldl, X + (int64_t)s1 * ldx, ldx,
                       1.0, X + (int64_t)s0 * ldx, ldx);
          if (rc) return rc;
        }
        rc = subst(h, true, L + (int64_t)s0 * ldl + s0, ldl, s1 - s0, X + (int64_t)s0 * ldx, ldx, n);
        if (rc) return rc;
      }
    }
  }
  return ISDF_OK;
}

int trsm_lower_right(isdf_handle h, bool trans, int m, int64_t n, const double* L, int64_t ldl, double* X, int64_t ldx) {
  ARG_CHECK(h, L && X && m > 0 && n > 0 && ldl >= m && ldx >= m);
  double* T = (double*)isdf_ws(h, "trsm_T", sizeof(double) * (size_t)m * (size_t)n);
  if (!T) return ISDF_ERR_HIP;
  int rc = transpose_rm(h, X, ldx, n, m, T, n);
  if (rc) return rc;
  rc = trsm_lower_left(h, !trans, m, n, L, ldl, T, n);
  if (rc) return rc;
  return transpose_rm(h, T, n, m, n, X, ldx);
}

namespace {
int trsm_block_size() {
  static const int nb = getenv("ISDF_TRSM_NB") ? std::max(64, atoi(getenv("ISDF_TRSM_NB"))) : 1024;
  return nb;
}
int rb_left(isdf_handle h, bool trans, int m, int64_t n, const double* L, int64_t ldl, double* X, int64_t ldx) {
  const double one = 1.0;
  ProfScope ps(h, "rocblas_dtrsm[flop]", (double)n * m * m);
  BLAS_TRY(h, rocblas_dtrsm(h->blas, rocblas_side_right, rocblas_fill_upper,
                            trans ? rocblas_operation_transpose : rocblas_operation_none, rocblas_diagonal_non_unit,
                            (rocblas_int)n, m, &one, L, (rocblas_int)ldl, X, (rocblas_int)ldx));
  return ISDF_OK;
}
// ... 73 lines not shown
```

### pyscf_isdf_amd/fit_route.py

```python
import numpy as np


class FitRouteMixin:
    def _bj_prepare(self, ao, nh, d_ip, ip_off, aoP, scratch=None):
        be = self.backend
        P = aoP.shape[0]
        be.gather_aoP(ao, d_ip, aoP)
        A = self._buffer('factor', (P, P))
        if getattr(self, '_psi', None) is not None and not nh:
            be.gram_prod(aoP, self._psiP, A)
        else:
            be.gram_sq(aoP, A, nh)
        self._Dinv_key = None
        be.shift_diag(A, self.reg_rel)
        Dblk = self._buffer('Dblk', (P, P))
        self.block_shift_used = be.block_chol(A, ip_off, self.block_shift, Dblk)
        be.block_solve(Dblk, ip_off, 0, 0, A)
        be.block_solve(Dblk, ip_off, 1, 1, A)
        extra = be.chol_inplace(A, 0.0, scratch=scratch)
        self.reg_used = self.reg_rel + extra
        return A, Dblk

    def _block_inverse(self, Dblk, ip_off):
        if not self.block_apply_mfma or int(np.diff(np.asarray(ip_off)).max()) > 1100:
            return None
        key = (Dblk.data_ptr(), getattr(self, '_build_serial', 0), len(ip_off))
        if getattr(self, '_Dinv_key', None) != key:
            Dinv = self._buffer('Dinv', tuple(Dblk.shape))
            self.backend.block_invert(Dblk, ip_off, Dinv)
            self._Dinv, self._Dinv_key = Dinv, key
        return self._Dinv

    def _bj_rows(self, aoP, nh, ao, ng, Dblk, ip_off, out):
        be = self.backend
        Dinv = self._block_inverse(Dblk, ip_off)
        if getattr(self, '_psi', None) is not None and not nh:
            be.pair_prod_rows(aoP, self._psiP, ao, self._psi, ng, out)
            if Dinv is not None:
                be.block_apply(Dinv, ip_off, out)
            else:
                be.block_solve(Dblk, ip_off, 0, 0, out)
            return
        if Dinv is not None and not nh:
            be.pair_rows_block_apply(aoP, ao, ng, Dinv, ip_off, out)
            return
        be.pair_gram_rows(aoP, ao, ng, out, nh)
        if Dinv is not None:
            be.block_apply(Dinv, ip_off, out)
        else:
            be.block_solve(Dblk, ip_off, 0, 0, out)

    def _resident_rows(self, G, P):
        if self.max_resident_rows:
            return int(self.max_resident_rows), int(self.max_resident_rows)
        be = self.backend
        have = be.free_bytes() + sum(int(b.numel()) * 8 for k, b in self._bufs.items() if k in ('theta', 'W', 'factor', 'Dblk', 'Dinv', 'rows_scratch'))
        if self.max_device_memory:
            have = min(have, int(self.max_device_memory) - sum(int(b.numel()) * 8 for k, b in self._bufs.items() if k in ('ao', 'psi')))
        fixed = 4 * 8 * P * P + (3 << 30)
        if getattr(self, 'pair_space', 'ao') == 'occ':
            nocc = min(self.cell.nao_nr() // 2, int(getattr(self.cell, 'nelectron', 0)) // 2 + 8)
            fixed += 8 * G * nocc + (2 << 30)
        fb = int(self.fft_batch or 0)
        single = (have - fixed - 24 * (min(128, fb) if fb else 128) * G) // (8 * G)
        panel = (have - fixed - 40 * (fb or 512) * G) // (8 * G)
        return max(0, int(single)), max(0, int(panel))

    def _panel_plan(self, ip_off, nrows_max):
        ip_off = np.asarray(ip_off, dtype=np.int64)
        P = int(ip_off[-1])
        big = int(np.diff(ip_off).max())
        if nrows_max < big:
            raise MemoryError('ISDF: not enough device memory for one block of %d fit rows' % big)
        npan = max(1, -(-P // int(nrows_max)))
        while True:
            cuts = [P]
            for k in range(npan - 1):
                want = max(cuts[-1] - int(nrows_max), 0)
                i0 = int(np.searchsorted(ip_off, want, side='left'))
                cand = [int(x) for x in ip_off[i0:] if x < cuts[-1] and x < want + 768]
                if not cand:
                    break
                b = min(cand, key=lambda x: ((-x) % 256, x)) if want > 0 else 0
                cuts.append(b)
            cuts.append(0)
            cuts = sorted(set(cuts))
            panels = [(x, y) for x, y in zip(cuts[:-1], cuts[1:]) if y > x]
            if all(y - x <= nrows_max for x, y in panels):
                return panels
            npan += 1

    def _bj_rows_range(self, r0, r1, out):
        be, st = self.backend, self._fit_state
        ip_off = np.asarray(st['ip_off'])
        i0, i1 = int(np.searchsorted(ip_off, r0)), int(np.searchsorted(ip_off, r1))
        assert ip_off[i0] == r0 and ip_off[i1] == r1
        G = self.ao.shape[1]
        Dinv = self._block_inverse(st['Dblk'], ip_off)
        sub = (ip_off[i0:i1 + 1] - r0).astype(np.int32)
        if getattr(self, '_psi', None) is not None:
            be.pair_prod_rows(self.aoP[r0:r1], self._psiP[r0:r1], self.ao, self._psi, G, out)
            if Dinv is not None:
                be.block_apply(Dinv[r0:r1, r0:r1], sub, out)
            else:
                be.block_solve(st['Dblk'][r0:r1, r0:r1], sub, 0, 0, out)
        elif Dinv is not None:
            be.pair_rows_block_apply(self.aoP[r0:r1], self.ao, G, Dinv[r0:r1, r0:r1], sub, out)
        else:
            be.pair_gram_rows(self.aoP[r0:r1], self.ao, G, out, 0)
            be.block_solve(st['Dblk'][r0:r1, r0:r1], sub, 0, 0, out)

    def _finish_W_paneled(self, W, probe=None):
        be, st = self.backend, self._fit_state
        cell = self.cell
        P = W.shape[0]
        mesh = np.asarray(self.mesh, dtype=np.int32)
        G = int(np.prod(mesh))
        a = np.asarray(cell.lattice_vectors(), dtype=float)
        w = cell.vol / G
        ip_off = np.asarray(st['ip_off'], dtype=np.int64)
        panels = st['panels']
        buf = st['rows']
        nbat = int(self.fft_batch or 512)
        big = int(np.diff(ip_off).max())
        self._last_fft_batch = nbat
        scratch = self._buffer('rows_scratch', (nbat + big, G))
        for q, (q0, q1) in enumerate(panels):
            Yq = buf[:q1 - q0]
            self._bj_rows_range(q0, q1, Yq)
            be.coulomb_W(Yq, mesh, a, 0, q1 - q0, min(nbat, q1 - q0), W[q0:q1, q0:q1], upper_only=True)
            if probe is not None:
                be.rows_combine(probe[0][:, q0:q1], Yq, probe[1], accumulate=q > 0)
            for p0, p1 in panels[:q]:
                nxt, fill, g0 = p0, 0, p0
                while nxt < p1 or fill > 0:
                    while fill < nbat and nxt < p1:
                        i = int(np.searchsorted(ip_off, nxt))
                        j = i + 1
                        while j + 1 < len(ip_off) and ip_off[j + 1] <= p1 and fill + (ip_off[j + 1] - nxt) <= nbat + big:
                            j += 1
                        b1 = int(ip_off[j])
                        self._bj_rows_range(nxt, b1, scratch[fill:fill + (b1 - nxt)])
                        fill += b1 - nxt
                        nxt = b1
                    take = min(nbat, fill)
                    V = scratch[:take]
                    be.coulomb_rows(V, mesh, a, take)
                    be.gemm_nt(V, Yq, W[g0:g0 + take, q0:q1], alpha=w)
                    if fill > take:
                        scratch[:fill - take].copy_(scratch[take:fill].clone() if fill - take > take else scratch[take:fill])
                    g0 += take
                    fill -= take
        be.symmetrize_upper(W)
        self._bj_finish(st['Afac'], st['Dblk'], st['ip_off'], W)

    def _spectral_plan(self):
        be = self.backend
        if not getattr(self, 'w_spectral', False) or not hasattr(be, 'spectral_rows'):
            return None
        mesh = np.asarray(self.mesh, dtype=np.int32)
        epoch = getattr(be, 'kernel_epoch', None)
        ckey = (tuple(int(x) for x in mesh), epoch, str(getattr(self, 'w_sphere', 'auto')), float(getattr(self, 'w_sphere_tol', 0.0)),
                int(self.fft_batch or 512), int(getattr(self, 'w_sort_bins', 0) or 0))
        cached = getattr(self, '_spectral_plan_cache', None)
        if epoch is not None and cached is not None and cached[0] == ckey:
            return cached[1]
        plan = self._spectral_plan_make(mesh)
        self._spectral_plan_cache = (ckey, plan)
        return plan

    def _spectral_plan_make(self, mesh):
        be = self.backend
        if not be.spectral_supported(mesh, int(self.fft_batch or 512)):
            return None
        a = np.asarray(self.cell.lattice_vectors(), dtype=float)
        G = int(np.prod(mesh))
        cg = be.coulG_half(mesh, a)
        if (cg < 0).any():
            return None
        w = self.cell.vol / G

        def share(pct, mult, box, keep):
            key = (tuple(int(x) for x in mesh), round(float(pct), 6))
            if getattr(self, '_sphere_share', (None,))[0] != key:
                self._sphere_share = (key, self._sphere_energy_share(mesh, cg, mult, box, keep, w))
            return self._sphere_share[1]
        pts = self._spectral_point_set(mesh, cg > 0, share)
        if pts is None:
            return None
        idx, mult = pts
        scale = np.sqrt(mult.ravel()[idx] * w * cg.ravel()[idx])
        npts = len(idx)
        ldx = -(-2 * npts // 128) * 128
        return dict(idx=be.to_device(idx), scale=be.to_device(scale), npts=npts, ldx=ldx, fraction=2.0 * npts / G)

    def _spectral_point_set(self, mesh, box, share):
        a = np.asarray(self.cell.lattice_vectors(), dtype=float)
        n0, n1, n2 = (int(x) for x in mesh)
        n2h = n2 // 2 + 1
        keep = box.copy()
        pct = getattr(self, 'w_sphere', 'auto')
        auto = isinstance(pct, str)
        pct = 100.0 if auto else float(pct or 0.0)
        if pct > 0:
            b = 2 * np.pi * np.linalg.inv(a).T
            f0, f1, f2 = np.fft.fftfreq(n0, 1.0 / n0), np.fft.fftfreq(n1, 1.0 / n1), np.arange(n2h, dtype=float)
            Gv = f0[:, None, None, None] * b[0] + f1[None, :, None, None] * b[1] + f2[None, None, :, None] * b[2]
            g2 = np.einsum('xyzc,xyzc->xyz', Gv, Gv)
            rmin = min(2 * np.pi * ((int(n) - 1) // 2) / np.linalg.norm(a[i]) for i, n in enumerate(mesh)) * pct / 100.0
            keep &= g2 <= rmin * rmin * (1 + 1e-12)
        mult = np.full((n0, n1, n2h), 2.0)
        mult[:, :, 0] = 1.0
        if n2 % 2 == 0:
            mult[:, :, n2 // 2] = 1.0
        if auto:
            if not (share(pct, mult, box, keep) <= float(getattr(self, 'w_sphere_tol', 1e-11))):
                return None
        idx = np.flatnonzero(keep.ravel()).astype(np.int32)
        if len(idx) == 0:
            return None
        nbins = int(getattr(self, 'w_sort_bins', 0) or 0)
        if nbins > 0:
            b = 2 * np.pi * np.linalg.inv(a).T
            f0, f1, f2 = np.fft.fftfreq(n0, 1.0 / n0), np.fft.fftfreq(n1, 1.0 / n1), np.arange(n2h, dtype=float)
            Gv = f0[:, None, None, None] * b[0] + f1[None, :, None, None] * b[1] + f2[None, None, :, None] * b[2]
            g2p = np.einsum('xyzc,xyzc->xyz', Gv, Gv).ravel()[idx]
            bins = np.minimum((g2p * (nbins / g2p.max())).astype(np.int64), nbins - 1)
            idx = idx[np.argsort(-bins, kind='stable')]
        return idx, mult

    def _sphere_energy_share(self, mesh, cg, mult, box, keep, w, ntest=8):
        import torch
        be = self.backend
        ao = getattr(self, 'ao', None)
        if ao is None:
            return np.inf
        nao, G = ao.shape
        rng = np.random.default_rng(7)
        cd = be.to_device(rng.standard_normal((2 * ntest, nao)) / np.sqrt(nao))
        rows = be.empty((2 * ntest, G))
        be.gemm_nn(cd, ao, rows)
        t = rows[:ntest].contiguous()
        be.hadamard_rows(t, rows[ntest:].contiguous())
        Gfull = int(np.prod(mesh))
        if G != Gfull:
            g0, g1 = self._slice
            full = be.zeros((ntest, Gfull))
            full[:, g0:g1] = t
            self.comm.all_reduce_sum(full)
            t = full
        idx = np.flatnonzero(box.ravel()).astype(np.int32)
        scale = np.sqrt(mult.ravel()[idx] * w * cg.ravel()[idx])
        ldx = -(-2 * len(idx) // 128) * 128
        X = be.empty((ntest, ldx))
        be.spectral_rows(t, mesh, be.to_device(idx), be.to_device(scale), X, batch=ntest)
        x = be.to_host(X)[:, :2 * len(idx)]
        e = x[:, 0::2] ** 2 + x[:, 1::2] ** 2
        outside = ~keep.ravel()[idx]
        tot = e.sum(axis=1)
        return float((e[:, outside].sum(axis=1) / np.where(tot > 0, tot, 1.0)).max())

    def _finish_W_spectral(self, W, probe=None):
        be, st = self.backend, self._fit_state
        plan = self._spectral_plan()
        ip_off = np.asarray(st['ip_off'], dtype=np.int64)
        P = W.shape[0]
        mesh = np.asarray(self.mesh, dtype=np.int32)
        G = int(np.prod(mesh))
        if plan is None:
            rows_avail = int(self._bufs['theta'].numel() // G)
            st2 = dict(st, kind='blockjacobi-paneled', rows=self._buffer('theta', (rows_avail, G)),
                       panels=self._panel_plan(ip_off, rows_avail))
            self._fit_state = st2
            try:
                return self._finish_W_paneled(W, probe=probe)
            finally:
                self._fit_state = st
        nbat = int(self.fft_batch or 512)
        big = int(np.diff(ip_off).max())
        self._last_fft_batch = nbat
        ldx = plan['ldx']
        X = self._buffer('theta', (P, ldx))
        piece = self._pair_rows_piece(big)
        scratch = self._buffer('rows_scratch', (nbat + big, G))
        self.w_spectral_fraction = plan['fraction']
        self._last_spectral_ldx = ldx
        if piece:
            self._spectral_rows_two_frontiers(X, scratch, piece, plan, probe)
            return self._spectral_W_finish(X, W, nbat)
        nxt, fill, g0 = 0, 0, 0
        while nxt < P or fill > 0:
            while fill < nbat and nxt < P:
                i = int(np.searchsorted(ip_off, nxt))
                j = i + 1
                while j + 1 < len(ip_off) and fill + (ip_off[j + 1] - nxt) <= nbat + big:
                    j += 1
                b1 = int(ip_off[j])
                self._bj_rows_range(nxt, b1, scratch[fill:fill + (b1 - nxt)])
                fill += b1 - nxt
                nxt = b1
            take = min(nbat, fill)
            rows = scratch[:take]
            if probe is not None:
                be.rows_combine(probe[0][:, g0:g0 + take], rows, probe[1], accumulate=g0 > 0)
            be.spectral_rows(rows, mesh, plan['idx'], plan['scale'], X[g0:g0 + take], batch=take)
            if fill > take:
                scratch[:fill - take].copy_(scratch[take:fill].clone() if fill - take > take else scratch[take:fill])
            g0 += take
            fill -= take
        self._spectral_W_finish(X, W, nbat)

    def _spectral_W_finish(self, X, W, nbat):
        be, st = self.backend, self._fit_state
        P = W.shape[0]
        for b0 in range(0, P, nbat):
            b1 = min(P, b0 + nbat)
            be.gemm_nt(X[b0:b1], X[b0:], W[b0:b1, b0:], alpha=1.0)
        be.symmetrize_upper(W)
        self._bj_finish(st['Afac'], st['Dblk'], st['ip_off'], W)

    def _pair_rows_piece(self, big):
        align = int(getattr(self, 'pair_rows_align', 0) or 0)
        if align <= 0 or not hasattr(self.backend, 'pair_rows_frontier') or getattr(self, '_psi', None) is not None \
                or not self.block_apply_mfma or big > 1100:
            return 0
        return int(self.fft_batch or 512) // align * align

    def _spectral_rows_two_frontiers(self, X, scratch, piece, plan, probe):
        be, st = self.backend, self._fit_state
        ip_off = np.asarray(st['ip_off'], dtype=np.int64)
        P = int(ip_off[-1])
        mesh = np.asarray(self.mesh, dtype=np.int32)
        G = self.ao.shape[1]
        Dinv = self._block_inverse(st['Dblk'], ip_off)
        nbat = int(self.fft_batch or 512)
        squared = be.pair_rows_squared(self.aoP, min(piece, P), self.ao, G)
        app, prod = 0, 0
        while app < P:
            new = min(piece, P - prod)
            j = int(np.searchsorted(ip_off, prod + new, side='right')) - 1
            i = int(np.searchsorted(ip_off, app))
            end = int(ip_off[j])
            be.pair_rows_frontier(self.aoP[prod:prod + new], self.ao, G, squared, Dinv[app:, app:],
                                  (ip_off[i:j + 1] - app).astype(np.int32), scratch, prod - app)
            prod += new
            if end > app:
                rows = scratch[:end - app]
                if probe is not None:
                    be.rows_combine(probe[0][:, app:end], rows, probe[1], accumulate=app > 0)
                be.spectral_rows(rows, mesh, plan['idx'], plan['scale'], X[app:end], batch=min(nbat, end - app))
                tail = prod - end
                if tail > 0:
                    src = scratch[end - app:prod - app]
                    scratch[:tail].copy_(src.clone() if tail > end - app else src)
                app = end

    def _bj_finish(self, Afac, Dblk, ip_off, W, antisymmetric=False):
        be = self.backend
        be.W_from_factor(Afac, 2, W)
        be.W_from_factor(Afac, 0, W)
        be.block_solve(Dblk, ip_off, 0, 1, W)
        be.block_solve(Dblk, ip_off, 1, 0, W)
        be.symmetrize_mean(W, antisymmetric)

    def _bj_clusters(self):
        cell = self.cell
        natm = cell.natm
        parent = list(range(natm))

        def find(i):
            while parent[i] != i:
                parent[i] = parent[parent[i]]
                i = parent[i]
            return i
        r = float(self.bj_cluster_radius or 0.0)
        if r > 0 and natm > 1:
            a = np.asarray(cell.lattice_vectors(), dtype=float)
            frac = np.asarray(cell.atom_coords(), dtype=float).dot(np.linalg.inv(a))
            d = frac[:, None, :] - frac[None, :, :]
            d -= np.round(d)
            dist = np.linalg.norm(d.dot(a), axis=2)
            for i, j in zip(*np.nonzero(np.triu(dist < r, 1))):
                ri, rj = find(int(i)), find(int(j))
                if ri != rj:
                    parent[max(ri, rj)] = min(ri, rj)
        groups = {}
        for i in range(natm):
            groups.setdefault(find(i), []).append(i)
        return [groups[k] for k in sorted(groups)]

    def _bj_blocks(self, counts, clusters):
        per = [int(sum(counts[b] for b in cl)) for cl in clusters]
        off = np.append(0, np.cumsum(per)).astype(np.int32)
        g = max(1, int(self.bj_group))
        if g > 1:
            off = np.unique(np.append(off[::g], off[-1])).astype(np.int32)
        return off

    def _fit_routes(self):
        if self.fit_route not in ('auto', 'blockjacobi', 'cholesky'):
            raise ValueError("fit_route must be 'auto', 'blockjacobi' or 'cholesky'")
        if self._want_theta or self.fit_route == 'cholesky':
            return ['cholesky']
        if self.fit_route == 'blockjacobi':
            return ['blockjacobi']
        if self.c_isdf > self.bj_max_c:
            return ['cholesky']
        return ['blockjacobi', 'cholesky']

    def _bj_probe_densities(self, aoT_P):
        be = self.backend
        planes = aoT_P if isinstance(aoT_P, (list, tuple)) else [aoT_P]
        nao, P = planes[0].shape
        n = int(self.bj_nprobe)
        if getattr(self, '_psi', None) is not None and len(planes) == 1:
            psiP = self._psiP
            nocc = psiP.shape[1]
            cached = getattr(self, '_probe_Rocc', None)
            if cached is None or cached[0] != (n, nao, nocc):
                rng = np.random.default_rng(20240203)
                self._probe_Rocc = ((n, nao, nocc), be.to_device(rng.standard_normal((n, nao, nocc))))
            d_R = self._probe_Rocc[1]
            aoP = planes[0].T.contiguous()
            ones = be.to_device(np.ones((nocc, 1)))
            T = be.empty((n, P))
            tmp = be.empty((P, nocc))
            col = be.empty((P, 1))
            for j in range(n):
                be.gemm_nn(aoP, d_R[j], tmp)
                be.hadamard_rows(tmp, psiP)
                be.gemm_nn(tmp, ones, col)
                T[j].copy_(col[:, 0])
            return T
# ... 55 lines not shown
```

### pyscf_isdf_amd/isdf.py

```python
import os
import sys
import time
import warnings
import numpy as np
import torch
from . import gto
from ._common import (UniformGrids, partition_grid_by_atom, _monkhorst_pack_size, _aoslice_by_atom,
                      _default_fft_batch)
from .fit_route import FitRouteMixin
from .sharded import ShardedMixin
from .kpoints import KPointMixin
from .hcore import HcoreMixin
from .eri_surface import EriSurfaceMixin
from .jk_e1 import JKE1Mixin
from .pp_grad import PPGradMixin


class ISDF(FitRouteMixin, ShardedMixin, KPointMixin, HcoreMixin, EriSurfaceMixin, JKE1Mixin, PPGradMixin):
    _keys = {'cell', 'kpts', 'grids', 'mesh', 'blockdim', 'exxdiv', 'c_isdf', 'select', 'tie_rtol'}

    def __init__(self, cell, kpts=np.zeros((1, 3)), c_isdf=12, select='refined', backend=None, comm=None):
        self.cell = cell
        self.stdout = getattr(cell, 'stdout', None) or sys.stdout
        self.verbose = getattr(cell, 'verbose', 0)
        self.max_memory = getattr(cell, 'max_memory', 4000)
        self.kpts_symm = None
        if hasattr(kpts, 'kpts_ibz') and hasattr(kpts, 'transform_dm'):
            self.kpts_symm = kpts
            kpts = kpts.kpts
        self.kpts = np.asarray(kpts).reshape(-1, 3)
        self.grids = UniformGrids(cell, cell.mesh)
        self.blockdim = 240
        self.exxdiv = None
        self.c_isdf = c_isdf
        self.select = select
        self.refine_over = 2.0
        self.pair_space = 'ao'
        self.occ_refit = 'always'
        self.w_spectral = True
        self.w_sphere = 'auto'
        self.w_sphere_tol = 1e-11
        self.w_sort_bins = 256
        self.w_spectral_check_tol = 5e-9
        self.w_spectral_max_c = 18
        self.cand_skip_zero_rows = True
        self.cand_gram = True
        self.cand_ao_cutoff = None
        self.tie_rtol = 1e-10
        self.select_tol = -1.0
        self.reg_rel = 1e-12
        self.reg_used = 0.0
        self.k_ip_factor = None
        self.kpt_pair_q = 'auto'
        self.kpt_w_spectral = False
        self.kpts_band = None
        self.force_sharded = False
        self.fit_route = 'auto'
        self.bj_check_tol = 3e-8
        self.bj_auto_kpts = False
        self.bj_max_c = 12
        self.bj_nprobe = 8
        self.bj_cluster_radius = 2.4
        self.bj_group = 1
        self.bj_check = None
        self.fit_route_used = None
        self.block_shift = 0.0
        self.block_shift_used = 0.0
        self.robust_k = False
        self.explicit_theta = False
        self.fft_batch = None
        self.pair_rows_align = 256
        self.block_apply_mfma = True
        self.max_resident_rows = None
        self.max_device_memory = None
        self.n_panels = 1
        self._backend = backend
        self._comm = comm
        self._rsh_df = {}
        self._built = False
        self._W_omega = {}
        self._fit_state = None
        self._fit_pending = False
        self._psi = self._psiP = None
        self._fit_dm = None
        self._V = None
        self._bufs = {}
        self._ovlp = None
        self.timings = {}
        self.ao = None
        self.aoP = None
        self.W = None
        self.ip = None

    @property
    def _want_theta(self):
        return bool(self.explicit_theta or self.robust_k)

    @property
    def _sharded(self):
        return self.comm.size > 1 or self.force_sharded or getattr(self.comm, 'always', False)

    @property
    def mesh(self):
        return self.grids.mesh

    @mesh.setter
    def mesh(self, mesh):
        self.grids.mesh = np.asarray(mesh)
        self.grids._coords = None

    @property
    def backend(self):
        if self._backend is None:
            from .backend import HipBackend
            dev = 0
            if self._comm is not None:
                dev = self._comm.local_rank
            if os.environ.get('ISDF_ONE_GPU'):
                dev = 0
            self._backend = HipBackend(dev)
        return self._backend

    def reset(self, cell=None):
        if cell is not None:
            self.cell = cell
# ... 885 lines not shown
```

### pyscf_isdf_amd/kpoints.py

```python
import time
import warnings
import numpy as np
import torch
from . import gto
from ._common import partition_grid_by_atom, _monkhorst_pack_size


class KPointMixin:
    def _get_k_exact_kpts(self, dm=None, mo_coeff=None, mo_occ=None, kpts_band=None, rows=None, max_rows=None):
        cell, be = self.cell, self.backend
        kpts = np.asarray(self.kpts, dtype=float).reshape(-1, 3)
        band = kpts if kpts_band is None else np.asarray(kpts_band, dtype=float).reshape(-1, 3)
        nk, nao = len(kpts), cell.nao_nr()
        mesh = np.asarray(self.mesh, dtype=np.int32)
        G = int(np.prod(mesh))
        a = np.asarray(cell.lattice_vectors(), dtype=float)
        if mo_coeff is None:
            mo_coeff, mo_occ = getattr(dm, 'mo_coeff', None), getattr(dm, 'mo_occ', None)
        orbs = []
        for k in range(nk):
            if mo_coeff is not None:
                orbs.append(self._orbitals_from_tag(mo_coeff[k], mo_occ[k]))
            else:
                orbs.append(self._orbitals_from_psd(np.asarray(dm).reshape(-1, nao, nao)[k]))
# ... 330 lines not shown
        Wim = self._buffer('Wim', (P, P))
        out, check = {}, 0.0
        for iq in st['primary']:
            if self._q_owner[iq] != comm.rank:
                continue
            q = self._qs[iq]
            coulG = be.coulG_q(mesh, cell.lattice_vectors(), q, omega=omega)
            if spec is not None:
                self._kspectral_Mq(spec, coulG, Wre, Wim)
            else:
                be.coulomb_Wq(Y, mesh, coulG, w, 0, P, st['batch'], Wre, Wim, upper_only=True)
                be.symmetrize_hermitian(Wre, Wim)
            jq = int(st['partner'][iq])
            twin = None
            if spec is not None:
                if self._pair_correct and jq >= 0 and jq != iq and not spec['pair_exact']:
                    twin = (be.empty((P, P)), be.empty((P, P)))
                    self._kspectral_Mq(spec, be.coulG_q(mesh, cell.lattice_vectors(), -np.asarray(q), omega=omega), twin[0], twin[1])
            elif self._pair_correct and jq >= 0 and jq != iq:
                twin = (be.empty((P, P)), be.empty((P, P)))
                twin[0].copy_(Wre)
                twin[1].copy_(Wim)
                twin[1].neg_()
                self._nyquist_pair_correction(q, omega, coulG, twin[0], twin[1])
            if st['route'] == 'blockjacobi':
                Afac, Dblk, ip_off = st['bj']
                self._bj_finish(Afac, Dblk, ip_off, Wre)
                self._bj_finish(Afac, Dblk, ip_off, Wim, antisymmetric=True)
                if probe and abs(q).max() < 1e-9:
                    t1 = self._tick('S4S5_coulomb_W', t0)
                    nao, nh, aoP_X = st['nao'], st['nh'], st['aoP_X']
                    planes = [aoP_X[:, o:o + nao].T.contiguous() for o in range(0, 2 * nh, nao)]
                    check = self._bj_probe_mismatch(planes, Afac, Dblk, ip_off, Y, G, None, W=Wre)
                    del planes
                    t0 = self._tick('S5_route_check', t1)
            elif not self._want_theta:
                be.W_from_factor(st['chol'], 0, Wre)
                be.W_from_factor(st['chol'], 0, Wim)
            Wc = be.empty((P, P), dtype=torch.complex128)
            be.finish_Wq(Wre, Wim, be.to_device(np.exp(-1j * r_ip.dot(q))), Wc)
            out[iq] = self._keep_Wq(Wc)
            del Wc
            if twin is not None:
                if st['route'] == 'blockjacobi':
                    self._bj_finish(Afac, Dblk, ip_off, twin[0])
                    self._bj_finish(Afac, Dblk, ip_off, twin[1], antisymmetric=True)
                elif not self._want_theta:
                    be.W_from_factor(st['chol'], 0, twin[0])
                    be.W_from_factor(st['chol'], 0, twin[1])
                Wt = be.empty((P, P), dtype=torch.complex128)
                be.finish_Wq(twin[0], twin[1], be.to_device(np.exp(1j * r_ip.dot(q))), Wt)
                out[jq] = self._keep_Wq(Wt)
                del twin, Wt
        return out, check, t0

    def _kspectral_prepare(self, Y):
        self.w_spectral_fraction = None
        if self.kpt_w_spectral is False:
            return None
        if self.kpt_w_spectral is not True:
            raise ValueError('kpt_w_spectral must be True or False')
        be = self.backend
        mesh = np.asarray(self.mesh, dtype=np.int32)
        nbat = int(self.fft_batch or 512)
        if not be.spectral_supported(mesh, nbat):
            return None
        n0, n1, n2 = (int(x) for x in mesh)
        pts = self._spectral_point_set(mesh, np.ones((n0, n1, n2 // 2 + 1), dtype=bool), self._ksphere_share)
        if pts is None:
            return None
        idx = pts[0]
        P, G = Y.shape
        npts = len(idx)
        ldx = -(-2 * npts // 128) * 128
        i2 = idx % (n2 // 2 + 1)
        i1 = (idx // (n2 // 2 + 1)) % n1
        i0 = idx // ((n2 // 2 + 1) * n1)
        on_nyq = np.zeros(npts, dtype=bool)
        for i, n in ((i0, n0), (i1, n1), (i2, n2)):
            if n % 2 == 0:
                on_nyq |= (i == n // 2)
        d_idx = be.to_device(idx)
        X = self._buffer('kspecX', (P, ldx))
        be.spectral_rows(Y, mesh, d_idx, be.to_device(np.ones(npts)), X, batch=nbat)
        self.w_spectral_fraction = 2.0 * npts / G
        return dict(X=X, idx=d_idx, npts=npts, ldx=ldx, pair_exact=not on_nyq.any(), strip=nbat,
                    s=self._buffer('kspec_s', (ldx,)), a=self._buffer('kspec_a', (ldx,)))

    def _ksphere_share(self, pct, mult, box, keep):
        mesh = np.asarray(self.mesh, dtype=np.int32)
        key = ('kpts', tuple(int(x) for x in mesh), round(float(pct), 6))
        if getattr(self, '_sphere_share', (None,))[0] != key:
            cg = self.backend.coulG_half(mesh, np.asarray(self.cell.lattice_vectors(), dtype=float))
            share = np.inf if (cg < 0).any() else \
                self._sphere_energy_share(mesh, cg, mult, box, keep, self.cell.vol / int(np.prod(mesh)))
            self._sphere_share = (key, share)
        return self._sphere_share[1]

    def _kspectral_Mq(self, spec, coulG, Mre, Mim):
        be = self.backend
        X = spec['X']
        P = X.shape[0]
        mesh = np.asarray(self.mesh, dtype=np.int32)
        G = int(np.prod(mesh))
        be.pack_table_pm(coulG, mesh, spec['idx'], self.cell.vol / G / G, spec['s'], spec['a'])
        nb = spec['strip']
        for b0 in range(0, P, nb):
            b1 = min(P, b0 + nb)
            be.herm_kscale_nt(X[b0:b1], X[b0:], spec['s'], spec['a'], Mre[b0:b1, b0:], Mim[b0:b1, b0:])
        be.symmetrize_hermitian(Mre, Mim)

    def _nyquist_planes(self):
        st = self._kfit_state
        if st.get('nyq') is not None:
            return st['nyq']
        be = self.backend
        Y = st['Y']
        P, G = Y.shape
        n = [int(x) for x in self.mesh]
        ii = [np.arange(m) for m in n]
        out = []
        for ax in range(3):
            if n[ax] % 2:
                continue
            oth = [i for i in range(3) if i != ax]
            A, B = np.meshgrid(ii[oth[0]], ii[oth[1]], indexing='ij')
            idx3 = [None, None, None]
            idx3[ax] = np.full(A.shape, n[ax] // 2)
            idx3[oth[0]], idx3[oth[1]] = A, B
            flat = ((idx3[0] * n[1] + idx3[1]) * n[2] + idx3[2]).ravel()
            neg = ((((-idx3[0]) % n[0]) * n[1] + ((-idx3[1]) % n[1])) * n[2] + ((-idx3[2]) % n[2])).ravel()
            fresh = np.ones(flat.shape, dtype=bool)
            for prev in range(ax):
                if n[prev] % 2 == 0:
                    fresh &= (idx3[prev].ravel() != n[prev] // 2)
            npl = len(flat)
            Tr, Ti = be.empty((P, npl)), be.empty((P, npl))
            nb = max(1, min(P, 65535, int((1 << 30) // (16 * npl))))
            for r0 in range(0, P, nb):
                r1 = min(P, r0 + nb)
                be.nyquist_spectra(Y[r0:r1], np.asarray(n, dtype=np.int32), ax, Tr[r0:r1], Ti[r0:r1])
            out.append(dict(Tr=Tr, Ti=Ti, flat=be.to_device(flat.astype(np.int64)), neg=be.to_device(neg.astype(np.int64)),
                            fresh=be.to_device(fresh.astype(np.float64))))
        st['nyq'] = out
        return out

    def _nyquist_pair_correction(self, q, omega, tab_q, Mre, Mim):
        cell, be = self.cell, self.backend
        mesh = np.asarray(self.mesh, dtype=np.int32)
        G = int(np.prod(mesh))
        w = cell.vol / G
        tab_m = be.coulG_q(mesh, cell.lattice_vectors(), -np.asarray(q), omega=omega)
        for pl in self._nyquist_planes():
            d = ((tab_m[pl['flat']] - tab_q[pl['neg']]) * pl['fresh']).contiguous()
            Tr, Ti = pl['Tr'], pl['Ti']
            P = Tr.shape[0]
            for r0 in range(0, P, 512):
                r1 = min(P, r0 + 512)
                be.gemm_nt(Tr[r0:r1], Tr[r0:], Mre[r0:r1, r0:], alpha=w / G, beta=1.0, kscale=d)
                be.gemm_nt(Ti[r0:r1], Ti[r0:], Mre[r0:r1, r0:], alpha=w / G, beta=1.0, kscale=d)
                be.gemm_nt(Ti[r0:r1], Tr[r0:], Mim[r0:r1, r0:], alpha=w / G, beta=1.0, kscale=d)
                be.gemm_nt(Tr[r0:r1], Ti[r0:], Mim[r0:r1, r0:], alpha=-w / G, beta=1.0, kscale=d)
        be.symmetrize_hermitian(Mre, Mim)
        del tab_m

    def _get_jk_kpts(self, dm, hermi, kpts, kpts_band, with_j, with_k, exxdiv, omega=None):
        ex = exxdiv if exxdiv is not None else self.exxdiv
# ... 238 lines not shown
```

### pyscf_isdf_amd/lib.py

```python
import ctypes
import os

_HERE = os.path.dirname(os.path.abspath(__file__))
LIB_PATH = os.path.join(_HERE, 'lib', 'libmi355_isdf.so')
ABI_VERSION = 21

_lib = None

c_int, c_i64, c_dbl, c_vp = ctypes.c_int, ctypes.c_int64, ctypes.c_double, ctypes.c_void_p

SIGNATURES = {
    'isdf_abi_version': (c_int, []),
    'isdf_create': (c_int, [c_int, ctypes.POINTER(c_vp)]),
    'isdf_destroy': (c_int, [c_vp]),
    'isdf_set_stream': (c_int, [c_vp, c_vp]),
    'isdf_last_error': (ctypes.c_char_p, [c_vp]),
    'isdf_workspace_bytes': (c_i64, [c_vp]),
    'isdf_set_coulomb_omega': (c_int, [c_vp, c_dbl]),
    'isdf_set_coulomb_cutoff': (c_int, [c_vp, c_dbl]),
    'isdf_set_coulomb_ws': (c_int, [c_vp, c_dbl, c_vp, c_vp, c_vp, c_vp]),
    'isdf_set_option': (c_int, [c_vp, ctypes.c_char_p, c_int]),
    'isdf_release_workspace': (c_int, [c_vp]),
    'isdf_prof_enable': (c_int, [c_vp, c_int]),
    'isdf_prof_reset': (c_int, [c_vp]),
    'isdf_prof_count': (c_int, [c_vp]),
    'isdf_prof_get': (c_int, [c_vp, c_int, ctypes.c_char_p, c_int, ctypes.POINTER(c_i64), ctypes.POINTER(c_dbl), ctypes.POINTER(c_dbl)]),
    'isdf_eval_ao': (c_int, [c_vp, c_vp, c_int, c_vp, c_int, c_vp, c_int, c_vp, c_int, c_vp, c_vp, c_i64, c_vp, c_i64]),
    'isdf_block_row_absmax': (c_int, [c_vp, c_vp, c_int, c_i64, c_int, c_vp, c_vp]),
    'isdf_gather_cols': (c_int, [c_vp, c_vp, c_int, c_i64, c_vp, c_i64, c_vp, c_i64]),
    'isdf_partition_by_atom': (c_int, [c_vp, c_vp, c_i64, c_vp, c_int, c_vp, c_dbl, c_vp]),
    'isdf_select_ip': (c_int, [c_vp, c_vp, c_int, c_i64, c_int, c_vp, c_vp, c_dbl, c_dbl, c_vp, c_i64, c_vp, c_vp]),
    'isdf_select_ip_ws': (c_int, [c_vp, c_vp, c_int, c_i64, c_int, c_vp, c_vp, c_dbl, c_dbl, c_vp, c_i64, c_vp, c_vp, c_vp,
                                  c_i64]),
    'isdf_select_ip_work_bytes': (c_i64, [c_int, c_i64]),
    'isdf_select_ip_gram': (c_int, [c_vp, c_vp, c_int, c_i64, c_int, c_dbl, c_dbl, c_int, c_vp, ctypes.POINTER(ctypes.c_int32)]),
    'isdf_fit_from_chol': (c_int, [c_vp, c_vp, c_int, c_i64, c_i64, c_vp]),
    'isdf_fit_prepare': (c_int, [c_vp, c_vp, c_int, c_i64, c_vp, c_int, c_dbl, c_vp, c_vp, ctypes.POINTER(c_dbl)]),
    'isdf_fit_apply': (c_int, [c_vp, c_vp, c_vp, c_int, c_int, c_vp, c_i64, c_i64, c_int, c_vp, c_i64]),
    'isdf_gather_aoP': (c_int, [c_vp, c_vp, c_int, c_i64, c_vp, c_int, c_vp]),
    'isdf_gram_sq': (c_int, [c_vp, c_vp, c_int, c_int, c_int, c_vp]),
    'isdf_pair_gram_rows': (c_int, [c_vp, c_vp, c_int, c_int, c_int, c_vp, c_i64, c_i64, c_vp, c_i64]),
    'isdf_gram_prod': (c_int, [c_vp, c_vp, c_int, c_int, c_vp, c_int, c_vp]),
    'isdf_pair_prod_rows': (c_int, [c_vp, c_vp, c_int, c_int, c_vp, c_int, c_vp, c_i64, c_vp, c_i64, c_i64, c_vp, c_i64]),
    'isdf_factor_solve_half': (c_int, [c_vp, c_vp, c_int, c_int, c_vp, c_i64, c_i64]),
    'isdf_gram_prod_cplx': (c_int, [c_vp, c_vp, c_int, c_int, c_int, c_vp, c_int, c_int, c_vp]),
    'isdf_pair_prod_rows_cplx': (c_int, [c_vp, c_vp, c_int, c_int, c_int, c_vp, c_int, c_int, c_vp, c_i64, c_vp, c_i64, c_i64,
                                         c_vp, c_i64]),
    'isdf_block_chol': (c_int, [c_vp, c_vp, c_int, c_int, c_vp, c_dbl, c_vp, ctypes.POINTER(c_dbl)]),
    'isdf_block_solve': (c_int, [c_vp, c_vp, c_int, c_int, c_vp, c_int, c_int, c_vp, c_i64, c_i64]),
    'isdf_block_invert': (c_int, [c_vp, c_vp, c_int, c_int, c_vp, c_vp]),
    'isdf_block_apply': (c_int, [c_vp, c_vp, c_i64, c_int, c_vp, c_vp, c_i64, c_i64]),
    'isdf_pair_rows_block_apply': (c_int, [c_vp, c_vp, c_int, c_int, c_vp, c_i64, c_i64, c_vp, c_i64, c_int, c_vp, c_vp, c_i64]),
    'isdf_pair_rows_squared': (c_int, [c_vp, c_vp, c_int, c_int, c_vp, c_i64, c_i64, ctypes.POINTER(c_int)]),
    'isdf_pair_rows_frontier': (c_int, [c_vp, c_vp, c_int, c_int, c_vp, c_i64, c_i64, c_int, c_vp, c_i64, c_int, c_vp, c_vp, c_i64,
                                        c_int]),
    'isdf_shift_diag': (c_int, [c_vp, c_vp, c_int, c_dbl]),
    'isdf_chol_inplace': (c_int, [c_vp, c_vp, c_int, c_dbl, c_vp, ctypes.POINTER(c_dbl)]),
    'isdf_factor_solve': (c_int, [c_vp, c_vp, c_int, c_vp, c_i64, c_i64]),
    'isdf_bj_probe_vectors': (c_int, [c_vp, c_vp, c_int, c_vp, c_vp, c_int, c_int, c_vp]),
    'isdf_rows_combine': (c_int, [c_vp, c_vp, c_int, c_i64, c_int, c_vp, c_i64, c_i64, c_vp, c_i64, c_int]),
    'isdf_bj_probe_rows': (c_int, [c_vp, c_vp, c_int, c_vp, c_vp, c_int, c_int, c_vp, c_vp, c_i64, c_i64, c_vp, c_i64]),
    'isdf_gather_T': (c_int, [c_vp, c_vp, c_int, c_i64, c_vp, c_vp]),
    'isdf_W_from_factor': (c_int, [c_vp, c_vp, c_int, c_int, c_vp, c_i64]),
    'isdf_fit_global': (c_int, [c_vp, c_vp, c_int, c_i64, c_i64, c_vp, c_int, c_dbl, c_vp, c_i64, c_vp, ctypes.POINTER(c_dbl)]),
    'isdf_coulomb_W': (c_int, [c_vp, c_vp, c_int, c_i64, c_vp, c_vp, c_int, c_int, c_int, c_int, c_vp, c_i64]),
    'isdf_coulomb_rows': (c_int, [c_vp, c_vp, c_int, c_i64, c_vp, c_vp, c_int, c_vp, c_i64]),
    'isdf_symmetrize_upper': (c_int, [c_vp, c_vp, c_int, c_i64]),
    'isdf_symmetrize_mean': (c_int, [c_vp, c_vp, c_int, c_i64, c_int]),
    'isdf_get_j': (c_int, [c_vp, c_vp, c_int, c_i64, c_i64, c_vp, c_vp, c_vp, c_int, c_vp]),
    'isdf_rho': (c_int, [c_vp, c_vp, c_int, c_i64, c_i64, c_vp, c_int, c_vp, c_i64]),
    'isdf_coulomb_potential': (c_int, [c_vp, c_vp, c_int, c_i64, c_vp, c_vp]),
    'isdf_vj_from_vR': (c_int, [c_vp, c_vp, c_int, c_i64, c_i64, c_vp, c_int, c_i64, c_vp]),
    'isdf_eval_ao_k': (c_int, [c_vp, c_vp, c_int, c_vp, c_int, c_vp, c_int, c_vp, c_int, c_vp, c_vp, c_int, c_vp, c_i64, c_vp, c_vp, c_i64]),
    'isdf_select_ip_cplx': (c_int, [c_vp, c_vp, c_int, c_int, c_i64, c_int, c_vp, c_vp, c_dbl, c_dbl, c_vp, c_i64, c_vp, c_vp]),
    'isdf_fit_prepare_cplx': (c_int, [c_vp, c_vp, c_int, c_int, c_i64, c_vp, c_int, c_dbl, c_vp, c_vp, ctypes.POINTER(c_dbl)]),
    'isdf_fit_apply_cplx': (c_int, [c_vp, c_vp, c_vp, c_int, c_int, c_int, c_vp, c_i64, c_i64, c_int, c_vp, c_i64]),
    'isdf_coulG_q': (c_int, [c_vp, c_vp, c_vp, c_vp, c_int, c_dbl, c_vp]),
    'isdf_coulomb_Wq': (c_int, [c_vp, c_vp, c_int, c_i64, c_vp, c_vp, c_dbl, c_int, c_int, c_int, c_int, c_vp, c_vp, c_i64]),
    'isdf_symmetrize_hermitian': (c_int, [c_vp, c_vp, c_vp, c_int, c_i64]),
    'isdf_finish_Wq': (c_int, [c_vp, c_vp, c_vp, c_int, c_i64, c_vp, c_vp]),
    'isdf_get_k_pair': (c_int, [c_vp, c_vp, c_vp, c_vp, c_vp, c_int, c_int, c_dbl, c_vp]),
    'isdf_get_k_exact_kpt': (c_int, [c_vp, c_vp, c_vp, c_int, c_i64, c_vp, c_vp, c_int, c_i64, c_vp, c_vp, c_dbl, c_int, c_int, c_int, c_vp, c_vp]),
    'isdf_coulG_half': (c_int, [c_vp, c_vp, c_vp, c_vp]),
    'isdf_spectral_supported': (c_int, [c_vp, c_vp, c_int, ctypes.POINTER(c_int)]),
    'isdf_spectral_rows': (c_int, [c_vp, c_vp, c_int, c_i64, c_vp, c_vp, c_vp, c_int, c_int, c_vp, c_i64]),
    'isdf_coulomb_rows_q': (c_int, [c_vp, c_vp, c_int, c_i64, c_vp, c_vp, c_vp, c_vp]),
    'isdf_nyquist_spectra': (c_int, [c_vp, c_vp, c_int, c_i64, c_vp, c_int, c_vp, c_vp]),
    'isdf_zhadamard_planes': (c_int, [c_vp, c_vp, c_vp, c_i64, c_vp, c_vp, c_i64, c_int, c_i64]),
    'isdf_rho_k': (c_int, [c_vp, c_vp, c_vp, c_int, c_i64, c_i64, c_vp, c_vp, c_dbl, c_vp]),
    'isdf_vj_k': (c_int, [c_vp, c_vp, c_vp, c_int, c_i64, c_i64, c_vp, c_vp, c_vp]),
    'isdf_pp_local_potential': (c_int, [c_vp, c_int, c_vp, c_vp, c_vp, c_vp, c_vp]),
    'isdf_pp_projector_overlaps': (c_int, [c_vp, c_vp, c_int, c_vp, c_int, c_vp, c_int, c_vp, c_vp, c_vp, c_vp, c_int, c_vp, c_vp, c_vp]),
    'isdf_pp_local_force': (c_int, [c_vp, c_vp, c_int, c_i64, c_int, c_vp, c_vp, c_vp, c_vp, c_vp]),
    'isdf_pp_projector_overlaps_ip': (c_int, [c_vp, c_vp, c_int, c_vp, c_int, c_vp, c_int, c_vp, c_vp, c_vp, c_vp, c_int, c_vp, c_vp,
                                              c_vp]),
    'isdf_rowdot3': (c_int, [c_vp, c_int, c_i64, c_dbl, c_vp, c_i64, c_i64, c_vp, c_vp, c_i64, c_int, c_vp, c_i64]),
    'isdf_gemm_nn': (c_int, [c_vp, c_int, c_i64, c_int, c_dbl, c_vp, c_i64, c_vp, c_i64, c_dbl, c_vp, c_i64]),
    'isdf_hadamard_rows': (c_int, [c_vp, c_vp, c_i64, c_vp, c_i64, c_int, c_i64]),
    'isdf_eval_ao_deriv1': (c_int, [c_vp, c_vp, c_int, c_vp, c_int, c_vp, c_int, c_vp, c_int, c_vp, c_vp, c_i64, c_vp, c_i64, c_i64]),
    'isdf_eval_ao_deriv2': (c_int, [c_vp, c_vp, c_int, c_vp, c_int, c_vp, c_int, c_vp, c_int, c_vp, c_vp, c_i64, c_vp, c_i64, c_i64]),
    'isdf_gga_aow': (c_int, [c_vp, c_int, c_i64, c_vp, c_i64, c_i64, c_vp, c_i64, c_vp, c_i64, c_vp, c_i64, c_i64]),
    'isdf_eval_ao_k_deriv1': (c_int, [c_vp, c_vp, c_int, c_vp, c_int, c_vp, c_int, c_vp, c_int, c_vp, c_vp, c_int, c_vp, c_i64, c_vp, c_vp, c_i64, c_i64]),
    'isdf_uniform_grid': (c_int, [c_vp, c_vp, c_vp, c_vp]),
    'isdf_rho_pair': (c_int, [c_vp, c_vp, c_int, c_vp, c_int, c_i64, c_i64, c_vp, c_int, c_vp, c_i64]),
    'isdf_mg_embed_density': (c_int, [c_vp, c_vp, c_int, c_vp, c_dbl, c_vp, c_vp, c_int]),
    'isdf_mg_restrict_potential': (c_int, [c_vp, c_vp, c_int, c_vp, c_vp, c_dbl, c_vp]),
    'isdf_mg_coulomb_kernel': (c_int, [c_vp, c_vp, c_int, c_vp, c_vp]),
    'isdf_lda_exchange': (c_int, [c_vp, c_vp, c_i64, c_vp, c_vp]),
    'isdf_lda_vwn_add': (c_int, [c_vp, c_vp, c_i64, c_vp, c_vp]),
    'isdf_gga_b88': (c_int, [c_vp, c_vp, c_vp, c_i64, c_i64, c_vp, c_vp, c_vp, c_i64]),
    'isdf_xc_fused': (c_int, [c_vp, c_vp, c_vp, c_i64, c_i64, c_dbl, c_dbl, c_dbl, c_int, c_dbl, c_vp, c_vp, c_vp, c_i64]),
    'isdf_gga_lyp_polarised': (c_int, [c_vp, c_vp, c_vp, c_i64, c_i64, c_i64, c_dbl, c_int, c_vp, c_vp, c_vp, c_i64, c_i64]),
    'isdf_lda_exchange_fxc': (c_int, [c_vp, c_vp, c_i64, c_vp]),
    'isdf_lda_vwn_fxc_add': (c_int, [c_vp, c_vp, c_i64, c_vp]),
    'isdf_gga_b88_fxc': (c_int, [c_vp, c_vp, c_i64, c_i64, c_vp, c_i64, c_i64, c_int, c_vp, c_i64, c_i64, c_vp, c_i64]),
    'isdf_xc_fxc_apply': (c_int, [c_vp, c_int, c_vp, c_i64, c_i64, c_i64, c_vp, c_i64, c_i64, c_int, c_vp, c_i64, c_i64, c_int]),
    'isdf_dot': (c_int, [c_vp, c_vp, c_vp, c_i64, c_vp]),
    'isdf_gemm_nt': (c_int, [c_vp, c_int, c_int, c_i64, c_dbl, c_vp, c_i64, c_vp, c_i64, c_vp, c_dbl, c_vp, c_i64]),
    'isdf_gemm_nt_had3': (c_int, [c_vp, c_int, c_int, c_i64, c_dbl, c_vp, c_i64, c_vp, c_i64, c_vp, c_i64, c_i64, c_dbl, c_vp, c_i64,
                                  c_i64]),
    'isdf_gemm_nn_had': (c_int, [c_vp, c_int, c_i64, c_int, c_dbl, c_vp, c_i64, c_vp, c_i64, c_vp, c_i64, c_dbl, c_vp, c_i64]),
    'isdf_pack_table_pm': (c_int, [c_vp, c_vp, c_vp, c_vp, c_int, c_dbl, c_vp, c_vp, c_i64]),
    'isdf_herm_kscale_nt': (c_int, [c_vp, c_int, c_int, c_i64, c_dbl, c_vp, c_i64, c_vp, c_i64, c_vp, c_vp, c_dbl, c_vp, c_vp, c_i64]),
    'isdf_get_k_exact': (c_int, [c_vp, c_vp, c_int, c_i64, c_i64, c_vp, c_int, c_vp, c_vp, c_int, c_int, c_int, c_vp]),
    'isdf_get_k': (c_int, [c_vp, c_vp, c_int, c_int, c_vp, c_i64, c_int, c_int, c_vp, c_int, c_vp]),
}


def load():
    global _lib
    if _lib is not None:
        return _lib
    if not os.path.exists(LIB_PATH):
        raise RuntimeError(
            'libmi355_isdf.so not found at %s — build it with `python -c "import __graft_entry__ as g; '
            'g.build()"` or `make -C pyscf_isdf_amd/csrc`.  There is no CPU fallback.' % LIB_PATH)
    try:
        import torch
    except ImportError:
        pass
    lib = ctypes.CDLL(LIB_PATH, mode=ctypes.RTLD_GLOBAL)
    for name, (res, args) in SIGNATURES.items():
        fn = getattr(lib, name)
        fn.restype = res
        fn.argtypes = args
    v = lib.isdf_abi_version()
    if v != ABI_VERSION:
        raise RuntimeError('libmi355_isdf.so ABI version %d != binding version %d' % (v, ABI_VERSION))
    _lib = lib
    return lib


class IsdfError(RuntimeError):
    pass


class Handle:

    def __init__(self, device=0):
        self.lib = load()
        h = c_vp()
        rc = self.lib.isdf_create(int(device), ctypes.byref(h))
        if rc != 0 or not h.value:
            raise IsdfError('isdf_create(device=%d) failed with status %d (no MI355X visible?)' % (device, rc))
        self.h = h
        self.device = device

    def call(self, name, *args):
# ... 16 lines not shown
```

### pyscf_isdf_amd/sharded.py

```python
import time
import warnings
import numpy as np
import torch
from . import gto
from ._common import partition_grid_by_atom, _default_fft_batch


class ShardedMixin:
    def _bj_finish_sharded(self, Afac, Dblk, ip_off, W):
        be, comm = self.backend, self.comm
        P = W.shape[0]
        c0, c1 = comm.split_range(P)
        X = W[:, c0:c1].clone()
        W.zero_()
        if c1 > c0:
            be.factor_solve(Afac, X)
            W[:, c0:c1] = X
        comm.all_reduce_sum(W)
        if c1 > c0:
            X.copy_(W[c0:c1, :].T)
        W.zero_()
        if c1 > c0:
            be.factor_solve(Afac, X)
            be.block_solve(Dblk, ip_off, 0, 1, X)
# ... 304 lines not shown
                    out = exchange_and_convolve(t, t % nslot)
                    staged[t] = (out, be.record_event())
            if t >= 1:
                out, ev = staged.pop(t - 1)
                be.wait_event(ev)
                products(*out)
                consumed[t - 1] = be.record_event()
        del staged, consumed, pieces, full, recvV
        comm.all_reduce_sum(W)
        be.symmetrize_upper(W)
        if st['kind'] == 'blockjacobi':
            self._bj_finish_sharded(st['Afac'], st['Dblk'], st['ip_off'], W)
        elif st['kind'] == 'cholesky':
            be.W_from_factor(st['chol'], 0, W)

    def _finish_W_sharded_spectral(self, W, plan, probe=None):
        cell, be, comm = self.cell, self.backend, self.comm
        st = self._fit_state
        ip_off = np.asarray(st['ip_off'], dtype=np.int64)
        P = int(ip_off[-1])
        ng = self.ao.shape[1]
        R, rk = comm.size, comm.rank
        mesh = np.asarray(self.mesh, dtype=np.int32)
        G = int(np.prod(mesh))
        ldx = int(plan['ldx'])
        self.w_spectral_fraction = plan['fraction']
        self._last_spectral_ldx = ldx
        self._last_fft_batch = int(self.fft_batch or 512)
        slices = [comm.split_range(G, r) for r in range(R)]
        ks = [tuple(16 * x for x in comm.split_range(ldx // 16, r)) for r in range(R)]
        kw = ks[rk][1] - ks[rk][0]
        nbat = int(self.fft_batch or 512)
        big = int(np.diff(ip_off).max())
        nblk = len(ip_off) - 1
        cuts = [int(np.searchsorted(ip_off, P * r / R, side='left')) for r in range(R)] + [nblk]
        cuts = [min(max(c, 0), nblk) for c in cuts]
        plans = []
        for q in range(R):
            b0, b1 = cuts[q], max(cuts[q + 1], cuts[q])
            steps, i = [], b0
            while i < b1:
                j = i + 1
                while j < b1 and ip_off[j + 1] - ip_off[i] <= max(nbat, big):
                    j += 1
                steps.append((int(ip_off[i]), int(ip_off[j])))
                i = j
            plans.append(steps)
        nsteps = max(len(p) for p in plans)
        cap = max([hi - lo for p in plans for lo, hi in p] + [1])
        Xloc = be.empty((P, max(kw, 1)))
        rows_loc = be.empty((R * cap, ng))
        pieces = be.empty((cap * G,))
        full = be.empty((cap, G))
        Xb = be.empty((cap, ldx))
        recvX = be.empty((R * cap * max(kw, 1),))

        def views(flat, nrow_of, width_of):
            out, off = [], 0
            for q in range(R):
                n = nrow_of(q) * width_of(q)
                out.append(flat[off:off + n].view(nrow_of(q), width_of(q)))
                off += n
            return out
        first = True
        for t in range(nsteps):
            bat = [p[t] if t < len(p) else (0, 0) for p in plans]
            nrow = [hi - lo for lo, hi in bat]
            send = []
            for q, (lo, hi) in enumerate(bat):
                blockrows = rows_loc[q * cap:q * cap + (hi - lo)]
                if hi > lo:
                    self._bj_rows_range(lo, hi, blockrows)
                    if probe is not None:
                        be.rows_combine(probe[0][:, lo:hi], blockrows, probe[1], accumulate=not first)
                        first = False
                send.append(blockrows)
            mine = nrow[rk]
            recv = views(pieces, lambda q: mine, lambda q: slices[q][1] - slices[q][0])
            comm.all_to_all(recv, send)
            rows_full = full[:mine]
            for (s0, s1), piece in zip(slices, recv):
                rows_full[:, s0:s1] = piece
            if mine:
                be.spectral_rows(rows_full, mesh, plan['idx'], plan['scale'], Xb[:mine], batch=mine)
            got = views(recvX, lambda q: nrow[q], lambda q: kw)
            comm.all_to_all(got, [Xb[:mine, k0:k1].contiguous() for k0, k1 in ks])
            for q in range(R):
                if nrow[q]:
                    Xloc[bat[q][0]:bat[q][1]] = got[q]
        del pieces, full, Xb, recvX, rows_loc
        W.zero_()
        if kw > 0:
            for b0 in range(0, P, 512):
                b1 = min(P, b0 + 512)
                be.gemm_nt(Xloc[b0:b1], Xloc[b0:], W[b0:b1, b0:], alpha=1.0)
        del Xloc
        comm.all_reduce_sum(W)
        be.symmetrize_upper(W)
        self._bj_finish_sharded(st['Afac'], st['Dblk'], st['ip_off'], W)

    def _keep_V_for_robust_k_sharded(self, t0):
        if not self.robust_k:
            return
        cell, be, comm = self.cell, self.backend, self.comm
        theta = self._fit_state['theta']
        P, ng = theta.shape
        R, rk = comm.size, comm.rank
        mesh = np.asarray(self.mesh, dtype=np.int32)
        G = int(np.prod(mesh))
        a = np.asarray(cell.lattice_vectors(), dtype=float)
        slices = [comm.split_range(G, r) for r in range(R)]
        rows = [comm.split_range(P, r) for r in range(R)]
        nb = self.fft_batch or _default_fft_batch(G, max(1, P // R))
        nsteps = max(-(-(hi - lo) // nb) for lo, hi in rows)
        for t in range(nsteps):
            bat = [(min(lo + t * nb, hi), min(lo + (t + 1) * nb, hi)) for lo, hi in rows]
            nrow = [hi - lo for lo, hi in bat]
            send = [theta[lo:hi] for lo, hi in bat]
            recv = [be.empty((nrow[rk], s1 - s0)) for s0, s1 in slices]
            comm.all_to_all(recv, send)
            full = be.empty((nrow[rk], G))
            for (s0, s1), piece in zip(slices, recv):
                full[:, s0:s1] = piece
            del recv
            if nrow[rk]:
                be.coulomb_rows(full, mesh, a, max(1, nrow[rk]))
            send = [full[:, s0:s1].contiguous() for s0, s1 in slices]
            recv = [be.empty((nrow[q], ng)) for q in range(R)]
            comm.all_to_all(recv, send)
            del full, send
            for q in range(R):
                if nrow[q]:
                    theta[bat[q][0]:bat[q][1]] = recv[q]
            del recv
        self._V = theta
        self._fit_state = None
        self._tick('S5_conv_for_robust_k', t0)

    def _get_jk_sharded(self, d_dm, out_shape, with_j, with_k, exxdiv=None):
        cell, be, comm = self.cell, self.backend, self.comm
        nao = cell.nao_nr()
        nset = d_dm.shape[0]
        mesh = np.asarray(self.mesh, dtype=np.int32)
        G = int(np.prod(mesh))
        a = np.asarray(cell.lattice_vectors(), dtype=float)
        g0, g1 = self._slice
        vj = vk = None
        t0 = time.perf_counter()
        if with_j:
            rho = be.zeros((nset, G))
            rho_loc = be.empty((nset, g1 - g0))
            be.rho(self.ao, g1 - g0, d_dm, rho_loc)
            rho[:, g0:g1] = rho_loc
            comm.all_reduce_sum(rho)
            be.coulomb_potential(rho, mesh, a)
            d_vj = be.empty((nset, nao, nao))
            be.vj_from_vR(self.ao, g1 - g0, rho[:, g0:g1].contiguous(), d_vj)
            comm.all_reduce_sum(d_vj)
            t0 = self._tick('S6_get_j', t0)
            vj = be.to_host(d_vj).reshape(out_shape)
        if with_k:
            P = self.W.shape[0]
            r0, r1 = comm.split_range(P)
            d_vk = be.empty((nset, nao, nao))
            be.get_k(self.aoP, self.W, r0, r1 - r0, d_dm, d_vk)
            comm.all_reduce_sum(d_vk)
            if self.robust_k:
# ... 7 lines not shown
```

Measured before the change: 16.74.

## Restrict spectral FFT last axis to occupied lines and fuse gather-scale

```diff
diff --git a/include/mi355_isdf.h b/include/mi355_isdf.h
--- a/include/mi355_isdf.h
+++ b/include/mi355_isdf.h
@@ -164,6 +164,10 @@
 int isdf_spectral_supported(isdf_handle h, const int32_t mesh[3], int batch, int* ok);
 int isdf_spectral_rows(isdf_handle h, const double* d_in, int nrows, int64_t ld, const int32_t mesh[3], const int32_t* d_idx,
                        const double* d_scale, int npts, int batch, double* d_out, int64_t ldx);
+int isdf_spectral_rows_lines(isdf_handle h, const double* d_in, int nrows, int64_t ld, const int32_t mesh[3], const int32_t* d_idx,
+                             const double* d_scale, int npts, const int32_t* d_lines, int nlines, int nlines_pad, int tile,
+                             const int32_t* d_slot, const double* d_slot_scale, int batch, double* d_out, int64_t ldx);
+int isdf_spectral_lines_tile(isdf_handle h, const int32_t mesh[3], int* tile);
 int isdf_coulomb_rows(isdf_handle h, const double* d_in, int nrows, int64_t ld,
                       const int32_t mesh[3], const double a[9], int batch, double* d_out, int64_t ldo);
 int isdf_symmetrize_upper(isdf_handle h, double* d_W, int P, int64_t ldw);
diff --git a/pyscf_isdf_amd/backend.py b/pyscf_isdf_amd/backend.py
--- a/pyscf_isdf_amd/backend.py
+++ b/pyscf_isdf_amd/backend.py
@@ -415,12 +415,28 @@
         self.handle.call('isdf_coulG_half', _np_ptr(mesh), _np_ptr(a), self._p(out))
         return self.to_host(out).reshape(int(mesh[0]), int(mesh[1]), int(mesh[2]) // 2 + 1)
 
-    def spectral_rows(self, rows, mesh, idx, scale, out, batch=512):
+    def spectral_lines_tile(self, mesh):
+        tile = ctypes.c_int(0)
+        mesh = np.ascontiguousarray(mesh, dtype=np.int32)
+        self.handle.call('isdf_spectral_lines_tile', _np_ptr(mesh), ctypes.byref(tile))
+        return int(tile.value)
+
+    def spectral_rows(self, rows, mesh, idx, scale, out, batch=512, lines=None, slot=None, slot_scale=None, nlines=0):
         self._stream()
         mesh = np.ascontiguousarray(mesh, dtype=np.int32)
         assert rows.is_contiguous() and out.stride(1) == 1 and idx.dtype == torch.int32 and out.stride(0) % 2 == 0
-        self.handle.call('isdf_spectral_rows', self._p(rows), rows.shape[0], rows.stride(0), _np_ptr(mesh), self._p(idx),
-                         self._p(scale), int(idx.numel()), int(batch), self._p(out), out.stride(0))
+        if lines is None:
+            self.handle.call('isdf_spectral_rows', self._p(rows), rows.shape[0], rows.stride(0), _np_ptr(mesh), self._p(idx),
+                             self._p(scale), int(idx.numel()), int(batch), self._p(out), out.stride(0))
+            return
+        assert lines.dtype == torch.int32 and slot.dtype == torch.int32 and slot_scale.dtype == torch.float64
+        assert lines.is_contiguous() and slot.is_contiguous() and slot_scale.is_contiguous() and slot.dim() == 3
+        tile = slot.shape[2]
+        assert lines.numel() % 16 == 0 and 0 < nlines <= lines.numel() and slot_scale.shape == slot.shape
+        assert tuple(slot.shape) == (lines.numel() // tile, int(mesh[0]), tile)
+        self.handle.call('isdf_spectral_rows_lines', self._p(rows), rows.shape[0], rows.stride(0), _np_ptr(mesh), self._p(idx),
+                         self._p(scale), int(idx.numel()), self._p(lines), int(nlines), int(lines.numel()), int(tile), self._p(slot),
+                         self._p(slot_scale), int(batch), self._p(out), out.stride(0))
 
     def symmetrize_upper(self, W):
         self._stream()
diff --git a/pyscf_isdf_amd/csrc/common.h b/pyscf_isdf_amd/csrc/common.h
--- a/pyscf_isdf_amd/csrc/common.h
+++ b/pyscf_isdf_amd/csrc/common.h
@@ -71,6 +71,10 @@
 bool spectral_rows_own_supported(isdf_handle h, const int32_t mesh[3], int nb);
 int spectral_rows_own(isdf_handle h, const double* d_in, int nb, const int32_t mesh[3], const int32_t* d_idx, const double* d_scale,
                       int npts, double* d_out, int64_t ldx, HIP_vector_type<double, 2u>* zbuf);
+int spectral_lines_tile(const int32_t mesh[3]);
+int spectral_rows_lines_own(isdf_handle h, const double* d_in, int nb, const int32_t mesh[3], int npts, const int32_t* d_lines,
+                            int nlines_pad, const int32_t* d_slot, const double* d_slot_scale, double* d_out, int64_t ldx,
+                            HIP_vector_type<double, 2u>* zbuf);
 int conv_rows_q_own(isdf_handle h, const double* d_in, double* d_re, double* d_im, int nb, const int32_t mesh[3], const double* tab,
                     double2* zhalf, double2* zfull);
 int conv_rows_own(isdf_handle h, const double* d_in, double* d_out, int nb, const int32_t mesh[3], const double* cg,
@@ -133,7 +137,7 @@
 int trsm_lower_left(isdf_handle h, bool trans, int m, int64_t n, const double* L, int64_t ldl, double* X, int64_t ldx);
 int trsm_lower_right(isdf_handle h, bool trans, int m, int64_t n, const double* L, int64_t ldl, double* X, int64_t ldx);
 int block_forward_solve(isdf_handle h, const double* D, int64_t ldd, int nblk, const int32_t* blk_off_host, double* X,
-                        int64_t ldx, int64_t n);
+                        int64_t ldx, int64_t n, bool own_columns = false);
 int block_apply_inverse(isdf_handle h, const double* Dinv, int64_t ldd, int nblk, const int32_t* blk_off_host, double* X,
                         int64_t ldx, int64_t n, bool square_input = false);
 int transpose_rm(isdf_handle h, const double* src, int64_t lds, int64_t rows, int64_t cols, double* dst, int64_t ldd);
diff --git a/pyscf_isdf_amd/csrc/coulomb.hip b/pyscf_isdf_amd/csrc/coulomb.hip
--- a/pyscf_isdf_amd/csrc/coulomb.hip
+++ b/pyscf_isdf_amd/csrc/coulomb.hip
@@ -376,3 +376,40 @@
   }
   return ISDF_OK;
 }
+
+extern "C" int isdf_spectral_lines_tile(isdf_handle h, const int32_t mesh[3], int* tile) {
+  if (!h) return ISDF_ERR_ARG;
+  ARG_CHECK(h, mesh && tile && mesh[0] > 0);
+  *tile = spectral_lines_tile(mesh);
+  return ISDF_OK;
+}
+
+extern "C" int isdf_spectral_rows_lines(isdf_handle h, const double* d_in, int nrows, int64_t ld, const int32_t mesh[3],
+                                        const int32_t* d_idx, const double* d_scale, int npts, const int32_t* d_lines, int nlines,
+                                        int nlines_pad, int tile, const int32_t* d_slot, const double* d_slot_scale, int batch,
+                                        double* d_out, int64_t ldx) {
+  if (!h) return ISDF_ERR_ARG;
+  ARG_CHECK(h, mesh && d_lines && d_slot && d_slot_scale && nlines > 0 && nlines <= nlines_pad && nlines_pad % 16 == 0);
+  ARG_CHECK(h, mesh[0] > 0 && tile == spectral_lines_tile(mesh));
+  const int64_t total = (int64_t)mesh[1] * (mesh[2] / 2 + 1);
+  ARG_CHECK(h, nlines <= total);
+  if ((int64_t)nlines * 10 >= total * 9) return isdf_spectral_rows(h, d_in, nrows, ld, mesh, d_idx, d_scale, npts, batch, d_out, ldx);
+  ARG_CHECK(h, d_in && d_out && d_idx && d_scale && nrows >= 0 && batch > 0 && npts > 0);
+  const int64_t G = (int64_t)mesh[0] * mesh[1] * mesh[2];
+  const int64_t gc = (int64_t)mesh[0] * total;
+  ARG_CHECK(h, ld == G && npts <= gc);
+  if (nrows == 0) return ISDF_OK;
+  if (batch > nrows) batch = nrows;
+  if (!spectral_rows_own_supported(h, mesh, batch))
+    return isdf_fail(h, ISDF_ERR_ARG, "isdf_spectral_rows_lines: mesh %d x %d x %d is not covered by the plane FFT", mesh[0], mesh[1],
+                     mesh[2]);
+  double2* Z = (double2*)isdf_ws(h, "coul_Z", sizeof(double2) * (size_t)batch * gc);
+  if (!Z) return ISDF_ERR_HIP;
+  for (int r = 0; r < nrows; r += batch) {
+    const int nb = std::min(batch, nrows - r);
+    int rc = spectral_rows_lines_own(h, d_in + (int64_t)r * ld, nb, mesh, npts, d_lines, nlines_pad, d_slot, d_slot_scale,
+                                     d_out + (int64_t)r * ldx, ldx, Z);
+    if (rc) return rc;
+  }
+  return ISDF_OK;
+}
diff --git a/pyscf_isdf_amd/csrc/fft_conv.hip b/pyscf_isdf_amd/csrc/fft_conv.hip
--- a/pyscf_isdf_amd/csrc/fft_conv.hip
+++ b/pyscf_isdf_amd/csrc/fft_conv.hip
@@ -538,6 +538,49 @@
   }
 }
 
+template <int ZCT>
+__global__ __launch_bounds__(TPB) void strided_fft_lines_kernel(const double2* __restrict__ data, int64_t os, int64_t es, Axis ax,
+                                                                int ntile, const int32_t* __restrict__ lines,
+                                                                const int32_t* __restrict__ slot,
+                                                                const double* __restrict__ slot_scale, int npts,
+                                                                double2* __restrict__ out, int64_t ldx2) {
+  static_assert(TPB % ZCT == 0, "one slot per thread");
+  constexpr int KS = 2048 / TPB;
+  extern __shared__ double2 lds[];
+  const int n = ax.n;
+  double2* x = lds;
+  double2* tw = lds + n * ZCT;
+  for (int k = threadIdx.x; k < n; k += TPB) tw[k] = ax.tw[k];
+  const int64_t outer = blockIdx.x / ntile;
+  const int t = blockIdx.x % ntile;
+  const int l = lines[t * ZCT + (threadIdx.x & (ZCT - 1))];
+  const double2* base = data + outer * os + l;
+  if (l >= 0)
+    for (int c = threadIdx.x; c < n * ZCT; c += TPB) x[c] = base[(int64_t)(c / ZCT) * es];
+  const int64_t tile0 = (int64_t)t * n * ZCT;
+  int js[KS];
+#pragma unroll
+  for (int k = 0; k < KS; ++k) {
+    const int c = threadIdx.x + k * TPB;
+    js[k] = (c < n * ZCT) ? slot[tile0 + c] : -1;
+  }
+  __syncthreads();
+  fft_fast<-1, ZCT>(x, ax, ZCT, tw);
+  double2* o = out + outer * ldx2;
+  double sc[KS];
+#pragma unroll
+  for (int k = 0; k < KS; ++k) sc[k] = (js[k] >= 0) ? slot_scale[tile0 + threadIdx.x + k * TPB] : 0.0;
+#pragma unroll
+  for (int k = 0; k < KS; ++k)
+    if (js[k] >= 0) {
+      const double2 v = x[threadIdx.x + k * TPB];
+      const double s = sc[k];
+      o[js[k]] = make_double2(v.x * s, v.y * s);
+    }
+  if (t == 0)
+    for (int64_t j = npts + threadIdx.x; j < ldx2; j += TPB) o[j] = make_double2(0.0, 0.0);
+}
+
 constexpr int TPBP = 1024;
 constexpr int PLANE_ENTRIES = 10240;
 constexpr int PIPE_NT = 768;
@@ -1155,6 +1198,32 @@
   return ISDF_OK;
 }
 
+int spectral_lines_tile(const int32_t mesh[3]) { return fast_lines(mesh[0]); }
+
+int spectral_rows_lines_own(isdf_handle h, const double* d_in, int nb, const int32_t mesh[3], int npts, const int32_t* d_lines,
+                            int nlines_pad, const int32_t* d_slot, const double* d_slot_scale, double* d_out, int64_t ldx,
+                            double2* zbuf) {
+  const int n0 = mesh[0], n1 = mesh[1], n2 = mesh[2], n2h = n2 / 2 + 1;
+  Axis ax[3];
+  if (int rc = make_axes(h, mesh, ax, "spectral_rows_lines_own")) return rc;
+  const int64_t gc = (int64_t)n0 * n1 * n2h;
+  const PlaneGeo geo = plane_geometry(n1, n2, false);
+  const int FX = fast_lines(n0);
+  ARG_CHECK(h, geo.bytes && FX >= 1 && (int64_t)nb * n0 < 2147483647LL && nb <= 65535 && (ldx & 1) == 0 && ldx >= 2 * (int64_t)npts);
+  ARG_CHECK(h, d_lines && d_slot && d_slot_scale && nlines_pad >= 16 && nlines_pad % 16 == 0 &&
+                   (int64_t)nb * (nlines_pad / FX) < 2147483647LL);
+  ProfScope ps(h, "spectral_rows_own[byte]", (8.0 * (double)n0 * n1 * n2 + 8.0 * (double)ldx) * nb, 2);
+  if (int rc = launch_plane_fwd(h, d_in, zbuf, ax, geo, (int)((int64_t)nb * n0), PIPE_ANY)) return rc;
+  const int nt = nlines_pad / FX;
+  with_lines(FX, [&](auto z) {
+    strided_fft_lines_kernel<decltype(z)::value><<<dim3((unsigned)((int64_t)nb * nt)), dim3(TPB), sizeof(double2) * ((size_t)n0 * FX + n0),
+                                                   h->stream>>>(zbuf, gc, (int64_t)n1 * n2h, ax[0], nt, d_lines, d_slot, d_slot_scale,
+                                                                npts, (double2*)d_out, ldx / 2);
+  });
+  KERNEL_CHECK(h);
+  return ISDF_OK;
+}
+
 bool conv_rows_q_own_supported(isdf_handle h, const int32_t mesh[3], int nb) {
   if (!h->own_fft) return false;
   if (nb < 1 || nb > 65535 || (int64_t)nb * mesh[0] >= 2147483647LL) return false;
diff --git a/pyscf_isdf_amd/csrc/fit.hip b/pyscf_isdf_amd/csrc/fit.hip
--- a/pyscf_isdf_amd/csrc/fit.hip
+++ b/pyscf_isdf_amd/csrc/fit.hip
@@ -385,20 +385,19 @@
 }
 
 namespace {
-__global__ void block_identity_kernel(double* __restrict__ E, int P, const int32_t* __restrict__ blk_of_row) {
-  const int64_t i = (int64_t)blockIdx.x * blockDim.x + threadIdx.x;
-  if (i < (int64_t)P * P) E[i] = (i / P == i % P) ? 1.0 : 0.0;
-  (void)blk_of_row;
+__global__ void block_identity_kernel(double* __restrict__ E, int P, int n) {
+  const int i = blockIdx.x * blockDim.x + threadIdx.x;
+  if (i < n) E[(int64_t)i * P + i] = 1.0;
 }
 }
 
 extern "C" int isdf_block_invert(isdf_handle h, const double* d_D, int P, int nblk, const int32_t* blk_off, double* d_Dinv) {
   if (!h) return ISDF_ERR_ARG;
   ARG_CHECK(h, d_D && d_Dinv && blk_off && P > 0 && nblk > 0 && blk_off[0] == 0 && blk_off[nblk] <= P);
-  hipLaunchKernelGGL(block_identity_kernel, dim3((unsigned)cdiv((int64_t)P * P, 256)), dim3(256), 0, h->stream, d_Dinv, P,
-                     (const int32_t*)nullptr);
-  KERNEL_CHECK(h);
-  return block_forward_solve(h, d_D, P, nblk, blk_off, d_Dinv, P, P);
+  HIP_TRY(h, hipMemsetAsync(d_Dinv, 0, sizeof(double) * (size_t)P * (size_t)P, h->stream));
+  hipLaunchKernelGGL(block_identity_kernel, dim3((unsigned)cdiv(P, 256)), dim3(256), 0, h->stream, d_Dinv, P, P);
+  KERNEL_CHECK(h);
+  return block_forward_solve(h, d_D, P, nblk, blk_off, d_Dinv, P, P, true);
 }
 
 extern "C" int isdf_block_apply(isdf_handle h, const double* d_Dinv, int64_t ldd, int nblk, const int32_t* blk_off,
diff --git a/pyscf_isdf_amd/csrc/trsm.hip b/pyscf_isdf_amd/csrc/trsm.hip
--- a/pyscf_isdf_amd/csrc/trsm.hip
+++ b/pyscf_isdf_amd/csrc/trsm.hip
@@ -58,12 +58,12 @@
 
 __global__ __launch_bounds__(256) void block_forward_kernel(const double* __restrict__ D, int64_t ldd,
                                                             const int32_t* __restrict__ blk_off,
-                                                            double* __restrict__ X, int64_t ldx, int64_t n) {
+                                                            double* __restrict__ X, int64_t ldx, int64_t n, int own_columns) {
   const int b = blockIdx.y;
   const int off = blk_off[b], m = blk_off[b + 1] - off;
   if (m <= 0) return;
-  const int64_t c = (int64_t)blockIdx.x * 256 + threadIdx.x;
-  if (c >= n) return;
+  const int64_t c = (int64_t)blockIdx.x * 256 + threadIdx.x + (own_columns ? off : 0);
+  if (c >= (own_columns ? min(n, (int64_t)off + m) : n)) return;
   const double* Db = D + (int64_t)off * ldd + off;
   double* Xb = X + (int64_t)off * ldx + c;
   const int nsub = (m + 63) >> 6;
@@ -347,17 +347,22 @@
 }
 
 int block_forward_solve(isdf_handle h, const double* D, int64_t ldd, int nblk, const int32_t* blk_off_host, double* X,
-                        int64_t ldx, int64_t n) {
+                        int64_t ldx, int64_t n, bool own_columns) {
   ARG_CHECK(h, D && X && blk_off_host && nblk > 0 && n > 0 && nblk <= 65535);
   int32_t* d_off = (int32_t*)isdf_ws(h, "trsm_blk_off", sizeof(int32_t) * (size_t)(nblk + 1));
   if (!d_off) return ISDF_ERR_HIP;
   HIP_TRY(h, hipMemcpyAsync(d_off, blk_off_host, sizeof(int32_t) * (size_t)(nblk + 1), hipMemcpyHostToDevice, h->stream));
   double rows2 = 0.0;
-  for (int b = 0; b < nblk; ++b) rows2 += (double)(blk_off_host[b + 1] - blk_off_host[b]) * (blk_off_host[b + 1] - blk_off_host[b]);
-  ProfScope ps(h, "block_forward_kernel[byte]", 16.0 * (double)blk_off_host[nblk] * (double)n);
-  (void)rows2;
-  hipLaunchKernelGGL(block_forward_kernel, dim3((unsigned)cdiv(n, 256), (unsigned)nblk), dim3(256), 0, h->stream, D, ldd, d_off,
-                     X, ldx, n);
+  int64_t widest = 0;
+  for (int b = 0; b < nblk; ++b) {
+    rows2 += (double)(blk_off_host[b + 1] - blk_off_host[b]) * (blk_off_host[b + 1] - blk_off_host[b]);
+    widest = std::max<int64_t>(widest, blk_off_host[b + 1] - blk_off_host[b]);
+  }
+  if (own_columns && widest <= 0) return ISDF_OK;
+  const int64_t ncol = own_columns ? widest : n;
+  ProfScope ps(h, "block_forward_kernel[byte]", 16.0 * (own_columns ? rows2 : (double)blk_off_host[nblk] * (double)n));
+  hipLaunchKernelGGL(block_forward_kernel, dim3((unsigned)cdiv(ncol, 256), (unsigned)nblk), dim3(256), 0, h->stream, D, ldd, d_off,
+                     X, ldx, n, own_columns ? 1 : 0);
   KERNEL_CHECK(h);
   return ISDF_OK;
 }
diff --git a/pyscf_isdf_amd/fit_route.py b/pyscf_isdf_amd/fit_route.py
--- a/pyscf_isdf_amd/fit_route.py
+++ b/pyscf_isdf_amd/fit_route.py
@@ -1,4 +1,22 @@
 import numpy as np
+
+
+def spectral_line_plan(idx, scale, mesh, tile):
+    idx = np.asarray(idx, dtype=np.int64)
+    n0, n1, n2 = (int(x) for x in mesh)
+    per = n1 * (n2 // 2 + 1)
+    line, kx = idx % per, idx // per
+    real = np.unique(line)
+    lines = np.full(-(-len(real) // 16) * 16, -1, dtype=np.int32)
+    lines[:len(real)] = real
+    slot = np.full((len(lines), n0), -1, dtype=np.int32)
+    where = np.searchsorted(real, line)
+    slot[where, kx] = np.arange(len(idx), dtype=np.int32)
+    if np.count_nonzero(slot >= 0) != len(idx):
+        return None
+    slot = np.ascontiguousarray(slot.reshape(-1, tile, n0).transpose(0, 2, 1))
+    slot_scale = np.where(slot >= 0, np.asarray(scale, dtype=np.float64)[np.maximum(slot, 0)], 0.0)
+    return lines, slot, slot_scale, len(real)
 
 
 class FitRouteMixin:
@@ -161,7 +179,7 @@
         mesh = np.asarray(self.mesh, dtype=np.int32)
         epoch = getattr(be, 'kernel_epoch', None)
         ckey = (tuple(int(x) for x in mesh), epoch, str(getattr(self, 'w_sphere', 'auto')), float(getattr(self, 'w_sphere_tol', 0.0)),
-                int(self.fft_batch or 512), int(getattr(self, 'w_sort_bins', 0) or 0))
+                int(self.fft_batch or 512), int(getattr(self, 'w_sort_bins', 0) or 0), bool(getattr(self, 'w_spectral_lines', True)))
         cached = getattr(self, '_spectral_plan_cache', None)
         if epoch is not None and cached is not None and cached[0] == ckey:
             return cached[1]
@@ -192,7 +210,17 @@
         scale = np.sqrt(mult.ravel()[idx] * w * cg.ravel()[idx])
         npts = len(idx)
         ldx = -(-2 * npts // 128) * 128
-        return dict(idx=be.to_device(idx), scale=be.to_device(scale), npts=npts, ldx=ldx, fraction=2.0 * npts / G)
+        return dict(idx=be.to_device(idx), scale=be.to_device(scale), npts=npts, ldx=ldx, fraction=2.0 * npts / G,
+                    lines_kw=self._spectral_lines_kw(idx, scale, mesh))
+
+    def _spectral_lines_kw(self, idx, scale, mesh):
+        be = self.backend
+        if not hasattr(be, 'spectral_lines_tile') or not getattr(self, 'w_spectral_lines', True):
+            return {}
+        lp = spectral_line_plan(idx, scale, mesh, be.spectral_lines_tile(mesh))
+        if lp is None:
+            return {}
+        return dict(lines=be.to_device(lp[0]), slot=be.to_device(lp[1]), slot_scale=be.to_device(lp[2]), nlines=lp[3])
 
     def _spectral_point_set(self, mesh, box, share):
         a = np.asarray(self.cell.lattice_vectors(), dtype=float)
@@ -253,7 +281,7 @@
         scale = np.sqrt(mult.ravel()[idx] * w * cg.ravel()[idx])
         ldx = -(-2 * len(idx) // 128) * 128
         X = be.empty((ntest, ldx))
-        be.spectral_rows(t, mesh, be.to_device(idx), be.to_device(scale), X, batch=ntest)
+        be.spectral_rows(t, mesh, be.to_device(idx), be.to_device(scale), X, batch=ntest, **self._spectral_lines_kw(idx, scale, mesh))
         x = be.to_host(X)[:, :2 * len(idx)]
         e = x[:, 0::2] ** 2 + x[:, 1::2] ** 2
         outside = ~keep.ravel()[idx]
@@ -303,7 +331,7 @@
             rows = scratch[:take]
             if probe is not None:
                 be.rows_combine(probe[0][:, g0:g0 + take], rows, probe[1], accumulate=g0 > 0)
-            be.spectral_rows(rows, mesh, plan['idx'], plan['scale'], X[g0:g0 + take], batch=take)
+            be.spectral_rows(rows, mesh, plan['idx'], plan['scale'], X[g0:g0 + take], batch=take, **plan['lines_kw'])
             if fill > take:
                 scratch[:fill - take].copy_(scratch[take:fill].clone() if fill - take > take else scratch[take:fill])
             g0 += take
@@ -348,7 +376,7 @@
                 rows = scratch[:end - app]
                 if probe is not None:
                     be.rows_combine(probe[0][:, app:end], rows, probe[1], accumulate=app > 0)
-                be.spectral_rows(rows, mesh, plan['idx'], plan['scale'], X[app:end], batch=min(nbat, end - app))
+                be.spectral_rows(rows, mesh, plan['idx'], plan['scale'], X[app:end], batch=min(nbat, end - app), **plan['lines_kw'])
                 tail = prod - end
                 if tail > 0:
                     src = scratch[end - app:prod - app]
diff --git a/pyscf_isdf_amd/isdf.py b/pyscf_isdf_amd/isdf.py
--- a/pyscf_isdf_amd/isdf.py
+++ b/pyscf_isdf_amd/isdf.py
@@ -41,6 +41,7 @@
         self.w_sphere = 'auto'
         self.w_sphere_tol = 1e-11
         self.w_sort_bins = 256
+        self.w_spectral_lines = True
         self.w_spectral_check_tol = 5e-9
         self.w_spectral_max_c = 18
         self.cand_skip_zero_rows = True
diff --git a/pyscf_isdf_amd/kpoints.py b/pyscf_isdf_amd/kpoints.py
--- a/pyscf_isdf_amd/kpoints.py
+++ b/pyscf_isdf_amd/kpoints.py
@@ -436,7 +436,7 @@
                 on_nyq |= (i == n // 2)
         d_idx = be.to_device(idx)
         X = self._buffer('kspecX', (P, ldx))
-        be.spectral_rows(Y, mesh, d_idx, be.to_device(np.ones(npts)), X, batch=nbat)
+        be.spectral_rows(Y, mesh, d_idx, be.to_device(np.ones(npts)), X, batch=nbat, **self._spectral_lines_kw(idx, np.ones(npts), mesh))
         self.w_spectral_fraction = 2.0 * npts / G
         return dict(X=X, idx=d_idx, npts=npts, ldx=ldx, pair_exact=not on_nyq.any(), strip=nbat,
                     s=self._buffer('kspec_s', (ldx,)), a=self._buffer('kspec_a', (ldx,)))
diff --git a/pyscf_isdf_amd/lib.py b/pyscf_isdf_amd/lib.py
--- a/pyscf_isdf_amd/lib.py
+++ b/pyscf_isdf_amd/lib.py
@@ -84,6 +84,9 @@
     'isdf_coulG_half': (c_int, [c_vp, c_vp, c_vp, c_vp]),
     'isdf_spectral_supported': (c_int, [c_vp, c_vp, c_int, ctypes.POINTER(c_int)]),
     'isdf_spectral_rows': (c_int, [c_vp, c_vp, c_int, c_i64, c_vp, c_vp, c_vp, c_int, c_int, c_vp, c_i64]),
+    'isdf_spectral_rows_lines': (c_int, [c_vp, c_vp, c_int, c_i64, c_vp, c_vp, c_vp, c_int, c_vp, c_int, c_int, c_int, c_vp, c_vp,
+                                         c_int, c_vp, c_i64]),
+    'isdf_spectral_lines_tile': (c_int, [c_vp, c_vp, c_vp]),
     'isdf_coulomb_rows_q': (c_int, [c_vp, c_vp, c_int, c_i64, c_vp, c_vp, c_vp, c_vp]),
     'isdf_nyquist_spectra': (c_int, [c_vp, c_vp, c_int, c_i64, c_vp, c_int, c_vp, c_vp]),
     'isdf_zhadamard_planes': (c_int, [c_vp, c_vp, c_vp, c_i64, c_vp, c_vp, c_i64, c_int, c_i64]),
diff --git a/pyscf_isdf_amd/sharded.py b/pyscf_isdf_amd/sharded.py
--- a/pyscf_isdf_amd/sharded.py
+++ b/pyscf_isdf_amd/sharded.py
@@ -410,7 +410,7 @@
             for (s0, s1), piece in zip(slices, recv):
                 rows_full[:, s0:s1] = piece
             if mine:
-                be.spectral_rows(rows_full, mesh, plan['idx'], plan['scale'], Xb[:mine], batch=mine)
+                be.spectral_rows(rows_full, mesh, plan['idx'], plan['scale'], Xb[:mine], batch=mine, **plan['lines_kw'])
             got = views(recvX, lambda q: nrow[q], lambda q: kw)
             comm.all_to_all(got, [Xb[:mine, k0:k1].contiguous() for k0, k1 in ks])
             for q in range(R):
```

Measured after the change: 16.58 (median of 6 runs). -1.0%, faster.
